# EricLBuehler/mistral.rs

Measured on NVIDIA H100. Metric: decode_tok_s, higher is better.
Workload: dtype int8 activations x 4/6-bit ggml blocks (dp4a), f32 accumulate, bf16 I/O

## Files before the change

mistral.rs_b200/csrc/common.cuh:

```cuda
#pragma once
#include <cuda_bf16.h>
#include <cuda_fp16.h>
#include <cuda_runtime.h>
#include <stdint.h>

#define MRS_WARP 32

enum : int {
  MRS_Q4_0 = 2, MRS_Q4_1 = 3, MRS_Q5_0 = 6, MRS_Q5_1 = 7, MRS_Q8_0 = 8, MRS_Q8_1 = 9,
  MRS_Q2_K = 10, MRS_Q3_K = 11, MRS_Q4_K = 12, MRS_Q5_K = 13, MRS_Q6_K = 14
};
enum : int { MRS_F16 = 0, MRS_BF16 = 1, MRS_F32 = 2 };

struct __align__(4) block_q8_1 {
  __half2 ds;
  int8_t qs[32];
};
static_assert(sizeof(block_q8_1) == 36, "q8_1 layout");

__device__ __forceinline__ float warp_sum(float x) {
#pragma unroll
  for (int m = 16; m > 0; m >>= 1) x += __shfl_xor_sync(0xffffffffu, x, m);
  return x;
}
__device__ __forceinline__ float warp_max(float x) {
#pragma unroll
  for (int m = 16; m > 0; m >>= 1) x = fmaxf(x, __shfl_xor_sync(0xffffffffu, x, m));
  return x;
}

__device__ __forceinline__ uint32_t smem_u32(const void *p) {
  return (uint32_t)__cvta_generic_to_shared(p);
}

__device__ __forceinline__ float load_act(const void *p, int64_t i, int dtype) {
  if (dtype == MRS_BF16) return __bfloat162float(((const __nv_bfloat16 *)p)[i]);
  if (dtype == MRS_F16) return __half2float(((const __half *)p)[i]);
  return ((const float *)p)[i];
}
__device__ __forceinline__ void store_act(void *p, int64_t i, float v, int dtype) {
  if (dtype == MRS_BF16) ((__nv_bfloat16 *)p)[i] = __float2bfloat16_rn(v);
  else if (dtype == MRS_F16) ((__half *)p)[i] = __float2half_rn(v);
  else ((float *)p)[i] = v;
}
__device__ __forceinline__ void load_act8(const void *p, int64_t i, int dtype, float *out) {
  if (dtype == MRS_BF16) {
    const uint4 v = *(const uint4 *)((const __nv_bfloat16 *)p + i);
    const __nv_bfloat162 *h = (const __nv_bfloat162 *)&v;
#pragma unroll
    for (int k = 0; k < 4; k++) { const float2 t = __bfloat1622float2(h[k]); out[2 * k] = t.x; out[2 * k + 1] = t.y; }
  } else if (dtype == MRS_F16) {
    const uint4 v = *(const uint4 *)((const __half *)p + i);
    const __half2 *h = (const __half2 *)&v;
#pragma unroll
    for (int k = 0; k < 4; k++) { const float2 t = __half22float2(h[k]); out[2 * k] = t.x; out[2 * k + 1] = t.y; }
  } else {
    const float4 a = *(const float4 *)((const float *)p + i), b = *(const float4 *)((const float *)p + i + 4);
    out[0] = a.x; out[1] = a.y; out[2] = a.z; out[3] = a.w; out[4] = b.x; out[5] = b.y; out[6] = b.z; out[7] = b.w;
  }
}
__device__ __forceinline__ void unpack_act8(const uint4 &v, int dtype, float *out) {
  if (dtype == MRS_BF16) {
    const __nv_bfloat162 *h = (const __nv_bfloat162 *)&v;
#pragma unroll
    for (int k = 0; k < 4; k++) { const float2 t = __bfloat1622float2(h[k]); out[2 * k] = t.x; out[2 * k + 1] = t.y; }
  } else {
    const __half2 *h = (const __half2 *)&v;
#pragma unroll
    for (int k = 0; k < 4; k++) { const float2 t = __half22float2(h[k]); out[2 * k] = t.x; out[2 * k + 1] = t.y; }
  }
}
__device__ __forceinline__ float round_act(float v, int dtype) {
  if (dtype == MRS_BF16) return __bfloat162float(__float2bfloat16_rn(v));
  if (dtype == MRS_F16) return __half2float(__float2half_rn(v));
  return v;
}

__device__ __forceinline__ float glu_activation(float x, int act) {
  switch (act) {
  case 1: {
    const float x3 = x * x * x;
    const float inner = 0.7978845608f * (x + 0.044715f * x3);
    float th;
    asm("tanh.approx.f32 %0, %1;" : "=f"(th) : "f"(inner));
    return 0.5f * x * (1.0f + th);
  }
  case 2: return fmaxf(x, 0.0f);
  case 3: return x * normcdff(x);
  case 4: return __fdividef(1.0f, 1.0f + __expf(-x));
  case 0:
  default: return __fdividef(x, 1.0f + __expf(-x));
  }
}

__device__ __forceinline__ void mbar_init(uint64_t *bar, uint32_t count) {
  asm volatile("mbarrier.init.shared::cta.b64 [%0], %1;" ::"r"(smem_u32(bar)), "r"(count));
}
__device__ __forceinline__ void fence_mbar_init() {
  asm volatile("fence.mbarrier_init.release.cluster;" ::: "memory");
}
__device__ __forceinline__ void fence_proxy_async() {
  asm volatile("fence.proxy.async.shared::cta;" ::: "memory");
}
__device__ __forceinline__ void mbar_arrive(uint64_t *bar) {
  asm volatile("mbarrier.arrive.shared::cta.b64 _, [%0];" ::"r"(smem_u32(bar)) : "memory");
}
__device__ __forceinline__ void mbar_arrive_expect_tx(uint64_t *bar, uint32_t bytes) {
  asm volatile("mbarrier.arrive.expect_tx.shared::cta.b64 _, [%0], %1;" ::"r"(smem_u32(bar)),
               "r"(bytes)
               : "memory");
}
__device__ __forceinline__ void mbar_wait(uint64_t *bar, uint32_t parity) {
  asm volatile(
      "{\n\t"
      ".reg .pred P1;\n\t"
      "WAIT_LOOP:\n\t"
      "mbarrier.try_wait.parity.shared::cta.b64 P1, [%0], %1;\n\t"
      "@P1 bra.uni WAIT_DONE;\n\t"
      "bra.uni WAIT_LOOP;\n\t"
      "WAIT_DONE:\n\t"
      "}" ::"r"(smem_u32(bar)),
      "r"(parity)
      : "memory");
}
__device__ __forceinline__ void bulk_g2s(void *dst_smem, const void *src_gmem, uint32_t bytes,
                                         uint64_t *bar) {
  asm volatile(
      "cp.async.bulk.shared::cluster.global.mbarrier::complete_tx::bytes [%0], [%1], %2, [%3];" ::
          "r"(smem_u32(dst_smem)),
      "l"(src_gmem), "r"(bytes), "r"(smem_u32(bar))
      : "memory");
}
__device__ __forceinline__ void pdl_wait() { asm volatile("griddepcontrol.wait;" ::: "memory"); }
__device__ __forceinline__ void pdl_launch_dependents() {
  asm volatile("griddepcontrol.launch_dependents;" ::: "memory");
}

__device__ __forceinline__ uint4 lds128(uint32_t saddr) {
  uint4 v;
  asm volatile("ld.shared.v4.u32 {%0, %1, %2, %3}, [%4];" : "=r"(v.x), "=r"(v.y), "=r"(v.z), "=r"(v.w) : "r"(saddr));
  return v;
}
__device__ __forceinline__ uint32_t lds32(uint32_t saddr) {
  uint32_t v;
  asm volatile("ld.shared.u32 %0, [%1];" : "=r"(v) : "r"(saddr));
  return v;
}
__device__ __forceinline__ uint32_t lds_u16s(uint32_t saddr) {
  uint16_t v;
  asm volatile("ld.shared.u16 %0, [%1];" : "=h"(v) : "r"(saddr));
  return (uint32_t)v;
}
__device__ __forceinline__ void sts128(uint32_t saddr, const uint4 &v) {
  asm volatile("st.shared.v4.u32 [%0], {%1, %2, %3, %4};" ::"r"(saddr), "r"(v.x), "r"(v.y), "r"(v.z), "r"(v.w) : "memory");
}
__device__ __forceinline__ void sts32(uint32_t saddr, uint32_t v) {
  asm volatile("st.shared.u32 [%0], %1;" ::"r"(saddr), "r"(v) : "memory");
}

__device__ __forceinline__ uint32_t lds_u32_unaligned(const uint8_t *p) {
  const uintptr_t a = (uintptr_t)p;
  const uint32_t *w = (const uint32_t *)(a & ~(uintptr_t)3);
  const uint32_t sh = (uint32_t)(a & 3) * 8;
  return __funnelshift_r(w[0], w[1], sh);
}
template <int N>
__device__ __forceinline__ void lds_words_unaligned(const uint8_t *p, uint32_t (&out)[N]) {
  const uintptr_t a = (uintptr_t)p;
  const uint32_t *w = (const uint32_t *)(a & ~(uintptr_t)3);
  const uint32_t sh = (uint32_t)(a & 3) * 8;
  uint32_t t[N + 1];
#pragma unroll
  for (int i = 0; i <= N; i++) t[i] = w[i];
#pragma unroll
  for (int i = 0; i < N; i++) out[i] = __funnelshift_r(t[i], t[i + 1], sh);
}
__device__ __forceinline__ uint32_t lds_u16(const uint8_t *p) {
  return *(const uint16_t *)p;
}

__device__ __forceinline__ float half_bits_to_float(uint32_t h16) {
  return __half2float(__ushort_as_half((unsigned short)h16));
}
```

mistral.rs_b200/csrc/decoder.cu:

```cuda
#include "common.cuh"
#include "dequant.cuh"
#include "mrs_b200_model.h"

#include <stdio.h>

extern "C" int mrs_mmvq_fused(int ggml_type, int mode, int dt, const void *w0, const void *w1, const void *w2,
                              const void *x, const void *norm_w, float eps, const void *residual, void *dst0,
                              void *dst1, void *dst2, int K, int n0, int n1, int n2, int b_size, int activation,
                              int pdl, void *stream);
extern "C" int mrs_mmvq_fused_qkv_mixed(int type_qk, int type_v, int dt, const void *wq, const void *wk, const void *wv,
                                        const void *x, const void *norm_w, float eps, void *q, void *k, void *v,
                                        int K, int nq, int nk, int nv, int b_size, int pdl, void *stream);
extern "C" void rotary_embedding_positions(void *query, void *key, void *cos_cache, void *sin_cache, void *positions,
                                           int32_t is_neox, int32_t head_size, int64_t num_tokens, int32_t rot_dim,
                                           int32_t seq_len, int32_t num_heads, int32_t num_kv_heads,
                                           int64_t query_stride, int64_t key_stride, uint32_t dtype, int64_t stream);
extern "C" void reshape_and_cache_flashinfer(void *key, void *value, void *key_cache, void *value_cache,
                                             int64_t *slot_mapping, int32_t num_tokens, int32_t num_heads,
                                             int32_t head_size, int32_t block_size, int32_t key_stride,
                                             int32_t value_stride, float k_scale, float v_scale, uint32_t dtype,
                                             uint32_t cache_dtype, cudaStream_t stream);
extern "C" int32_t mrs_paged_decode_fused(void *q, void *k_new, void *v_new, void *key_cache, void *value_cache,
                                          const void *rope_cos, const void *rope_sin, const int32_t *positions,
                                          const int64_t *slot_mapping, const int32_t *kv_indptr,
                                          const int32_t *kv_indices, const int32_t *kv_last_page_len,
                                          const int32_t *request_indices, const int32_t *kv_tile_indices,
                                          const int32_t *o_indptr, const int32_t *kv_chunk_size_ptr,
                                          const uint8_t *block_valid_mask, void *o, void *tmp_v, float *tmp_s,
                                          int32_t *counters, int32_t batch_size, int32_t padded_batch_size,
                                          int32_t num_qo_heads, int32_t num_kv_heads, int32_t head_size,
                                          int32_t page_size, float sm_scale, uint32_t dtype, int32_t pdl,
                                          void *stream);
extern "C" int32_t flashinfer_decode(void *q, void *key_cache, void *value_cache, const int32_t *kv_indptr,
                                     const int32_t *kv_indices, const int32_t *kv_last_page_len,
                                     const int32_t *request_indices, const int32_t *kv_tile_indices,
                                     const int32_t *o_indptr, const int32_t *kv_chunk_size_ptr,
                                     const bool *block_valid_mask, void *o, void *tmp_v, void *tmp_s,
                                     int32_t batch_size, int32_t padded_batch_size, int32_t num_qo_heads,
                                     int32_t num_kv_heads, int32_t head_size, int32_t page_size, int32_t q_stride_n,
                                     int32_t q_stride_h, float sm_scale, int32_t window_left, float logits_soft_cap,
                                     float k_scale, float v_scale, uint32_t dtype, uint32_t cache_dtype,
                                     cudaStream_t stream);

namespace mrs {

__global__ void embedding_gather_kernel(int type, const uint8_t *__restrict__ table, int cols,
                                        const int32_t *__restrict__ ids, void *__restrict__ out, int act_dtype) {
  const int row = ids[blockIdx.x];
  const int be = blk_elems(type), bb = blk_bytes(type);
  const uint8_t *rp = table + (size_t)row * (cols / be) * bb;
  for (int i = threadIdx.x; i < cols; i += blockDim.x)
    store_act(out, (int64_t)blockIdx.x * cols + i, dequant_elem(type, rp + (size_t)(i / be) * bb, i % be), act_dtype);
}

__device__ __forceinline__ unsigned long long pack_key(float v, int idx) {
  unsigned int b = __float_as_uint(v);
  b = (b & 0x80000000u) ? ~b : (b | 0x80000000u);
  return ((unsigned long long)b << 32) | (unsigned int)(0xFFFFFFFFu - (unsigned int)idx);
}
__global__ void argmax_kernel(const void *__restrict__ logits, int cols, int act_dtype, int32_t *__restrict__ out,
                              unsigned long long *__restrict__ keys, unsigned int *__restrict__ counts, int pdl) {
  __shared__ unsigned long long sk[32];
  if (pdl) pdl_wait();
  const int row = blockIdx.y;
  const int64_t base = (int64_t)row * cols;
  unsigned long long best = 0ull;
  for (int i = blockIdx.x * blockDim.x + threadIdx.x; i < cols; i += gridDim.x * blockDim.x) {
    const unsigned long long k = pack_key(load_act(logits, base + i, act_dtype), i);
    best = k > best ? k : best;
  }
#pragma unroll
  for (int m = 16; m > 0; m >>= 1) {
    const unsigned long long o = __shfl_xor_sync(0xffffffffu, best, m);
    best = o > best ? o : best;
  }
  const int w = threadIdx.x >> 5, l = threadIdx.x & 31;
  if (l == 0) sk[w] = best;
  __syncthreads();
  if (w == 0) {
    best = (l < (blockDim.x >> 5)) ? sk[l] : 0ull;
#pragma unroll
    for (int m = 16; m > 0; m >>= 1) {
      const unsigned long long o = __shfl_xor_sync(0xffffffffu, best, m);
      best = o > best ? o : best;
    }
    if (l == 0) {
      atomicMax(&keys[row], best);
      __threadfence();
      const unsigned int done = atomicAdd(&counts[row], 1u);
      if (done == gridDim.x - 1) {
        __threadfence();
        const unsigned long long k = atomicExch(&keys[row], 0ull);
        out[row] = (int32_t)(0xFFFFFFFFu - (unsigned int)(k & 0xFFFFFFFFull));
        counts[row] = 0u;
      }
    }
  }
}

__global__ void add_residual_kernel(void *__restrict__ dst, const void *__restrict__ res, int64_t n, int dt) {
  const int64_t i = (int64_t)blockIdx.x * blockDim.x + threadIdx.x;
  if (i < n) store_act(dst, i, load_act(dst, i, dt) + load_act(res, i, dt), dt);
}

struct ArCtxDev {
  int world, rank;
  const uint8_t *peer_base[8];
  uint32_t *flags_local;
  unsigned long long flags_off, slot_off[2];
  uint32_t *seq;
  unsigned long long ll_off, ll_slot_stride, ll_src_stride;
};
__global__ void __launch_bounds__(1024) tp_allreduce_residual_kernel(const ArCtxDev c, int slot, const void *__restrict__ residual,
                                                                     void *__restrict__ out, int count, int dt, int pdl) {
  __shared__ uint32_t s_seq;
  if (pdl && threadIdx.x == 0) pdl_launch_dependents();
  if (pdl) pdl_wait();
  if (threadIdx.x == 0) {
    const uint32_t seq = *c.seq + 1u;
    *c.seq = seq;
    __threadfence_system();
    for (int r = 0; r < c.world; r++) {
      uint32_t *flag = (uint32_t *)(c.peer_base[r] + c.flags_off) + c.rank;
      asm volatile("st.release.sys.global.u32 [%0], %1;" ::"l"(flag), "r"(seq) : "memory");
    }
    for (int r = 0; r < c.world; r++) {
      uint32_t v;
      do {
        asm volatile("ld.acquire.sys.global.u32 %0, [%1];" : "=r"(v) : "l"(c.flags_local + r) : "memory");
      } while ((int32_t)(v - seq) < 0);
    }
    s_seq = seq;
  }
  __syncthreads();
  for (int i = threadIdx.x * 8; i < count; i += blockDim.x * 8) {
    float acc[8] = {0.f, 0.f, 0.f, 0.f, 0.f, 0.f, 0.f, 0.f};
    for (int r = 0; r < c.world; r++) {
      const uint4 raw = __ldcv((const uint4 *)(c.peer_base[r] + c.slot_off[slot]) + (i >> 3));
      float v[8];
      unpack_act8(raw, dt, v);
#pragma unroll
      for (int k = 0; k < 8; k++) acc[k] += v[k];
    }
    float res[8];
    load_act8(residual, i, dt, res);
#pragma unroll
    for (int k = 0; k < 8; k++) store_act(out, (int64_t)i + k, round_act(acc[k], dt) + res[k], dt);
  }
}

__global__ void __launch_bounds__(1024) tp_allreduce_ll_kernel(const ArCtxDev c, int slot, const void *__restrict__ partial,
                                                               const void *__restrict__ residual, void *__restrict__ out, int count,
                                                               int dt, int pdl) {
  if (pdl && threadIdx.x == 0) pdl_launch_dependents();
  if (pdl) pdl_wait();
  const uint32_t seq = *(volatile const uint32_t *)c.seq + 1u;
  const bool dead = *(volatile const uint32_t *)(c.seq + 1) != 0u;
  __syncthreads();
  if (threadIdx.x == 0) *(volatile uint32_t *)c.seq = seq;
  const unsigned long long area = c.ll_off + (unsigned long long)slot * c.ll_slot_stride;
  const int npairs = count >> 1;
  for (int i = threadIdx.x; i < npairs; i += blockDim.x) {
    const uint32_t mine = ((const uint32_t *)partial)[i];
    for (int r = 0; r < c.world; r++) {
      if (r == c.rank) continue;
      uint2 *dst = (uint2 *)(c.peer_base[r] + area + (unsigned long long)c.rank * c.ll_src_stride) + i;
      asm volatile("st.volatile.global.v2.u32 [%0], {%1, %2};" ::"l"(dst), "r"(mine), "r"(seq) : "memory");
    }
  }
  for (int i = threadIdx.x; i < npairs; i += blockDim.x) {
    const uint32_t mine = ((const uint32_t *)partial)[i];
    float a0 = 0.f, a1 = 0.f;
    for (int r = 0; r < c.world; r++) {
      uint32_t w = mine;
      if (r != c.rank) {
        const uint2 *src = (const uint2 *)(c.peer_base[c.rank] + area + (unsigned long long)r * c.ll_src_stride) + i;
        uint32_t fl, spins = 0;
        const long long t0 = clock64();
        for (;;) {
          asm volatile("ld.volatile.global.v2.u32 {%0, %1}, [%2];" : "=r"(w), "=r"(fl) : "l"(src) : "memory");
          if (fl == seq || dead) break;
          if ((++spins & 1023u) == 0u &&
              (clock64() - t0 > 500000000ll || *(volatile const uint32_t *)(c.seq + 1) != 0u)) { c.seq[1] = 1u; break; }
        }
      }
      float v0, v1;
      if (dt == MRS_BF16) { const float2 f = __bfloat1622float2(*(const __nv_bfloat162 *)&w); v0 = f.x; v1 = f.y; }
      else { const float2 f = __half22float2(*(const __half2 *)&w); v0 = f.x; v1 = f.y; }
      a0 += v0; a1 += v1;
    }
    const float r0 = load_act(residual, 2 * (int64_t)i, dt), r1 = load_act(residual, 2 * (int64_t)i + 1, dt);
    store_act(out, 2 * (int64_t)i, round_act(a0, dt) + r0, dt);
    store_act(out, 2 * (int64_t)i + 1, round_act(a1, dt) + r1, dt);
  }
}

constexpr int ADV_MAX_BATCH = 256;
__global__ void decode_advance_kernel(const int32_t *__restrict__ block_tables, int max_blocks,
                                      int32_t *__restrict__ context_lens, int batch, int bs, int split_pages,
                                      int padded_tiles, int max_pos, int32_t *positions, int64_t *slot_mapping,
                                      int32_t *kv_indptr, int32_t *kv_indices, int32_t *kv_last_page_len,
                                      int32_t *request_indices, int32_t *kv_tile_indices, int32_t *o_indptr,
                                      int32_t *kv_chunk_size, uint8_t *block_valid_mask, int32_t *error_flag) {
  __shared__ int s_nb[ADV_MAX_BATCH], s_chunks[ADV_MAX_BATCH], s_indptr[ADV_MAX_BATCH + 1], s_oind[ADV_MAX_BATCH + 1];
  const int cap = min(max_blocks * bs, max_pos > 0 ? max_pos : max_blocks * bs);
  for (int b = threadIdx.x; b < batch; b += blockDim.x) {
    int pos = context_lens[b];
    const bool full = pos >= cap;
    if (full) { pos = cap - 1; if (error_flag != nullptr) atomicOr(error_flag, 1); }
    const int ctx = pos + 1;
    context_lens[b] = ctx;
    positions[b] = pos;
    slot_mapping[b] = full ? (int64_t)-1 : (int64_t)block_tables[(int64_t)b * max_blocks + pos / bs] * bs + pos % bs;
    const int nb = (ctx + bs - 1) / bs;
    s_nb[b] = nb;
    kv_last_page_len[b] = ctx - (nb - 1) * bs;
    s_chunks[b] = (split_pages > 0) ? ((nb < 1 ? 1 : nb) + split_pages - 1) / split_pages : 1;
  }
  __syncthreads();
  if (threadIdx.x == 0) {
    int nnz = 0, tiles = 0;
    s_indptr[0] = 0; s_oind[0] = 0;
    for (int b = 0; b < batch; b++) {
      nnz += s_nb[b];
      tiles = min(tiles + s_chunks[b], padded_tiles);
      s_indptr[b + 1] = nnz; s_oind[b + 1] = tiles;
    }
    kv_chunk_size[0] = (split_pages > 0 ? split_pages : 1) * bs;
  }
  __syncthreads();
  const int tiles = s_oind[batch];
  for (int b = threadIdx.x; b <= batch; b += blockDim.x) { kv_indptr[b] = s_indptr[b]; o_indptr[b] = s_oind[b]; }
  for (int b = 0; b < batch; b++) {
    const int t0 = s_oind[b], nt = s_oind[b + 1] - t0;
    for (int t = threadIdx.x; t < nt; t += blockDim.x) { request_indices[t0 + t] = b; kv_tile_indices[t0 + t] = t; }
    const int p0 = s_indptr[b], nb = s_indptr[b + 1] - p0;
    for (int i = threadIdx.x; i < nb; i += blockDim.x) kv_indices[p0 + i] = block_tables[(int64_t)b * max_blocks + i];
  }
  for (int t = threadIdx.x; t < padded_tiles; t += blockDim.x) {
    block_valid_mask[t] = t < tiles ? 1 : 0;
    if (t >= tiles) { request_indices[t] = 0; kv_tile_indices[t] = 0; }
  }
}

}

using namespace mrs;

extern "C" int32_t mrs_embedding_gather(int32_t ggml_type, const void *table, int32_t cols, const int32_t *ids,
                                        int32_t n, void *out, int32_t act_dtype, void *stream) {
  if (n <= 0) return 0;
  if (blk_bytes(ggml_type) == 0 || cols % blk_elems(ggml_type)) return (int32_t)cudaErrorInvalidValue;
  embedding_gather_kernel<<<n, 256, 0, (cudaStream_t)stream>>>(ggml_type, (const uint8_t *)table, cols, ids, out, act_dtype);
  return (int32_t)cudaGetLastError();
}

extern "C" int32_t mrs_argmax(const void *logits, int32_t rows, int32_t cols, int32_t act_dtype, int32_t *out,
                              void *scratch, int32_t pdl, void *stream) {
  if (rows <= 0) return 0;
  if (scratch == nullptr) return (int32_t)cudaErrorInvalidValue;
  unsigned long long *keys = (unsigned long long *)scratch;
  unsigned int *counts = (unsigned int *)(keys + rows);
  int chunks = (cols + 4095) / 4096;
  if (chunks > 64) chunks = 64;
  cudaLaunchConfig_t cfg = {};
  cfg.gridDim = dim3(chunks, rows); cfg.blockDim = dim3(256); cfg.stream = (cudaStream_t)stream;
  cudaLaunchAttribute attr[1];
  attr[0].id = cudaLaunchAttributeProgrammaticStreamSerialization;
  attr[0].val.programmaticStreamSerializationAllowed = 1;
  cfg.attrs = attr; cfg.numAttrs = pdl ? 1 : 0;
  return (int32_t)cudaLaunchKernelEx(&cfg, argmax_kernel, logits, (int)cols, (int)act_dtype, out, keys, counts, (int)pdl);
}

extern "C" int32_t mrs_decode_advance(const int32_t *block_tables, int32_t max_blocks_per_seq, int32_t *context_lens,
                                      int32_t batch, int32_t block_size, int32_t split_pages, int32_t padded_tiles,
                                      int32_t *positions, int64_t *slot_mapping, int32_t *kv_indptr,
                                      int32_t *kv_indices, int32_t *kv_last_page_len, int32_t *request_indices,
                                      int32_t *kv_tile_indices, int32_t *o_indptr, int32_t *kv_chunk_size,
                                      uint8_t *block_valid_mask, int32_t max_pos, int32_t *error_flag, void *stream) {
  if (batch < 1 || batch > ADV_MAX_BATCH || max_blocks_per_seq < 1 || block_size < 1) return (int32_t)cudaErrorInvalidValue;
  decode_advance_kernel<<<1, 256, 0, (cudaStream_t)stream>>>(block_tables, max_blocks_per_seq, context_lens, batch,
                                                             block_size, split_pages, padded_tiles, max_pos, positions,
                                                             slot_mapping, kv_indptr, kv_indices, kv_last_page_len,
                                                             request_indices, kv_tile_indices, o_indptr, kv_chunk_size,
                                                             block_valid_mask, error_flag);
  return (int32_t)cudaGetLastError();
}

extern "C" int32_t mrs_tp_allreduce_residual(const mrs_tp_ctx *ctx, int32_t slot, const void *residual, void *out,
                                             int32_t count, int32_t dtype, int32_t pdl, void *stream) {
  if (ctx == nullptr || ctx->world < 1 || ctx->world > 8 || (slot & ~1) || count % 8 || (dtype != MRS_F16 && dtype != MRS_BF16))
    return (int32_t)cudaErrorInvalidValue;
  ArCtxDev c = {};
  c.world = ctx->world; c.rank = ctx->rank;
  for (int r = 0; r < ctx->world; r++) c.peer_base[r] = (const uint8_t *)ctx->peer_base[r];
  c.flags_off = (unsigned long long)ctx->flags_offset;
  c.slot_off[0] = (unsigned long long)ctx->slot_offset[0]; c.slot_off[1] = (unsigned long long)ctx->slot_offset[1];
  c.flags_local = (uint32_t *)((uint8_t *)ctx->peer_base[ctx->rank] + ctx->flags_offset);
  c.seq = (uint32_t *)ctx->seq_counter;
  c.ll_off = (unsigned long long)ctx->ll_offset; c.ll_slot_stride = (unsigned long long)ctx->ll_slot_stride;
  c.ll_src_stride = (unsigned long long)ctx->ll_src_stride;
  if (ctx->ll_offset != 0) {
    if ((int64_t)count * 4 > ctx->ll_src_stride) return (int32_t)cudaErrorInvalidValue;
    int th = (count / 2 + 31) / 32 * 32;
    if (th > 1024) th = 1024;
    cudaLaunchConfig_t cfg = {};
    cfg.gridDim = dim3(1); cfg.blockDim = dim3(th); cfg.stream = (cudaStream_t)stream;
    cudaLaunchAttribute attr[1];
    attr[0].id = cudaLaunchAttributeProgrammaticStreamSerialization;
    attr[0].val.programmaticStreamSerializationAllowed = 1;
    cfg.attrs = attr; cfg.numAttrs = pdl ? 1 : 0;
    const void *partial = (const uint8_t *)ctx->peer_base[ctx->rank] + ctx->slot_offset[slot];
    return (int32_t)cudaLaunchKernelEx(&cfg, tp_allreduce_ll_kernel, c, (int)slot, partial, residual, out, (int)count, (int)dtype, (int)pdl);
  }
  int threads = (count / 8 + 31) / 32 * 32;
  if (threads > 1024) threads = 1024;
  if (threads < 32) threads = 32;
  cudaLaunchConfig_t cfg = {};
  cfg.gridDim = dim3(1); cfg.blockDim = dim3(threads); cfg.stream = (cudaStream_t)stream;
  cudaLaunchAttribute attr[1];
  attr[0].id = cudaLaunchAttributeProgrammaticStreamSerialization;
  attr[0].val.programmaticStreamSerializationAllowed = 1;
  cfg.attrs = attr; cfg.numAttrs = pdl ? 1 : 0;
  return (int32_t)cudaLaunchKernelEx(&cfg, tp_allreduce_residual_kernel, c, (int)slot, residual, out, (int)count, (int)dtype, (int)pdl);
}

#define MRS_TRY(expr)                                  \
  do {                                                 \
    const int _e = (int)(expr);                        \
    if (_e != 0) {                                     \
      fprintf(stderr, "mrs_b200: %s -> cudaError %d\n", #expr, _e); \
      return _e;                                       \
    }                                                  \
  } while (0)

extern "C" int32_t mrs_llama_decode_step(const mrs_llama_step *s, void *stream) {
  const int dt = s->act_dtype, B = s->batch, H = s->hidden, pdl = s->pdl;
  const int nq = s->n_heads * s->head_dim, nkv = s->n_kv_heads * s->head_dim;
  cudaStream_t st = (cudaStream_t)stream;
  if (B < 1 || B > 8) return (int32_t)cudaErrorInvalidValue;
  const bool do_attn = !(s->skip_mask & 1), do_gemv = !(s->skip_mask & 2);

  MRS_TRY(mrs_embedding_gather(s->tok_embd.ggml_type, s->tok_embd.data, H, s->token_ids, B, s->x, dt, stream));
  void *hidden = s->x, *hidden2 = s->x2;
  for (int l = 0; l < s->n_layers; l++) {
    const mrs_llama_layer &L = s->layers[l];
    if (!do_gemv) {
    } else if (L.wq.ggml_type != L.wk.ggml_type) {
      MRS_TRY(mrs_mmvq_fused(L.wq.ggml_type, 0, dt, L.wq.data, nullptr, nullptr, hidden, L.attn_norm, s->rms_eps,
                             nullptr, s->q, nullptr, nullptr, H, nq, 0, 0, B, 0, pdl, stream));
      MRS_TRY(mrs_mmvq_fused(L.wk.ggml_type, 0, dt, L.wk.data, nullptr, nullptr, hidden, L.attn_norm, s->rms_eps,
                             nullptr, s->k, nullptr, nullptr, H, nkv, 0, 0, B, 0, pdl, stream));
      MRS_TRY(mrs_mmvq_fused(L.wv.ggml_type, 0, dt, L.wv.data, nullptr, nullptr, hidden, L.attn_norm, s->rms_eps,
                             nullptr, s->v, nullptr, nullptr, H, nkv, 0, 0, B, 0, pdl, stream));
    } else if (L.wk.ggml_type == L.wv.ggml_type) {
      MRS_TRY(mrs_mmvq_fused(L.wq.ggml_type, 2, dt, L.wq.data, L.wk.data, L.wv.data, hidden, L.attn_norm, s->rms_eps,
                             nullptr, s->q, s->k, s->v, H, nq, nkv, nkv, B, 0, pdl, stream));
    } else {
      MRS_TRY(mrs_mmvq_fused(L.wq.ggml_type, 2, dt, L.wq.data, L.wk.data, nullptr, hidden, L.attn_norm, s->rms_eps,
                             nullptr, s->q, s->k, nullptr, H, nq, nkv, 0, B, 0, pdl, stream));
      MRS_TRY(mrs_mmvq_fused(L.wv.ggml_type, 0, dt, L.wv.data, nullptr, nullptr, hidden, L.attn_norm, s->rms_eps,
                             nullptr, s->v, nullptr, nullptr, H, nkv, 0, 0, B, 0, pdl, stream));
    }
    if (do_attn && s->fused_attention) {
      MRS_TRY(mrs_paged_decode_fused(s->q, s->k, s->v, L.k_cache, L.v_cache, s->rope_cos, s->rope_sin, s->positions,
                                     s->slot_mapping, s->kv_indptr, s->kv_indices, s->kv_last_page_len,
                                     s->request_indices, s->kv_tile_indices, s->o_indptr, s->kv_chunk_size,
                                     s->block_valid_mask, s->attn_out, s->padded_tiles > B ? s->tmp_v : nullptr,
                                     s->padded_tiles > B ? s->tmp_s : nullptr, s->attn_counters, B, s->padded_tiles,
                                     s->n_heads, s->n_kv_heads, s->head_dim, s->block_size, s->sm_scale, (uint32_t)dt,
                                     pdl | (s->rope_neox ? 0 : 2), stream));
    } else if (do_attn) {
    rotary_embedding_positions(s->q, s->k, (void *)s->rope_cos, (void *)s->rope_sin, s->positions, s->rope_neox,
                               s->head_dim, B, s->head_dim / 2, 0, s->n_heads, s->n_kv_heads, nq, nkv, (uint32_t)dt,
                               (int64_t)stream);
    reshape_and_cache_flashinfer(s->k, s->v, L.k_cache, L.v_cache, s->slot_mapping, B, s->n_kv_heads, s->head_dim,
                                 s->block_size, nkv, nkv, 1.f, 1.f, (uint32_t)dt, (uint32_t)dt, st);
    MRS_TRY(flashinfer_decode(s->q, L.k_cache, L.v_cache, s->kv_indptr, s->kv_indices, s->kv_last_page_len,
                              s->request_indices, s->kv_tile_indices, s->o_indptr, s->kv_chunk_size,
                              (const bool *)s->block_valid_mask, s->attn_out, s->padded_tiles > B ? s->tmp_v : nullptr,
                              s->padded_tiles > B ? s->tmp_s : nullptr, B, s->padded_tiles, s->n_heads, s->n_kv_heads,
                              s->head_dim, s->block_size, nq, s->head_dim, s->sm_scale, -1, 0.f, 1.f, 1.f,
                              (uint32_t)dt, (uint32_t)dt, st));
    }
    if (!do_gemv) continue;
    if (s->tp != nullptr && s->tp->world > 1) {
      void *part = (uint8_t *)s->tp->peer_base[s->tp->rank] + s->tp->slot_offset[0];
      MRS_TRY(mrs_mmvq_fused(L.wo.ggml_type, 0, dt, L.wo.data, nullptr, nullptr, s->attn_out, nullptr, 0.f, nullptr,
                             part, nullptr, nullptr, nq, H, 0, 0, B, 0, pdl, stream));
      MRS_TRY(mrs_tp_allreduce_residual(s->tp, 0, hidden, hidden2, B * H, dt, pdl, stream));
    } else if (s->all_reduce == nullptr) {
      MRS_TRY(mrs_mmvq_fused(L.wo.ggml_type, 0, dt, L.wo.data, nullptr, nullptr, s->attn_out, nullptr, 0.f, hidden,
                             hidden2, nullptr, nullptr, nq, H, 0, 0, B, 0, pdl, stream));
    } else {
      MRS_TRY(mrs_mmvq_fused(L.wo.ggml_type, 0, dt, L.wo.data, nullptr, nullptr, s->attn_out, nullptr, 0.f, nullptr,
                             hidden2, nullptr, nullptr, nq, H, 0, 0, B, 0, pdl, stream));
      s->all_reduce(hidden2, (int64_t)B * H, dt, stream, s->all_reduce_user);
      add_residual_kernel<<<(unsigned)(((int64_t)B * H + 255) / 256), 256, 0, st>>>(hidden2, hidden, (int64_t)B * H, dt);
    }
    if (L.w_gate.ggml_type != L.w_up.ggml_type || L.w_gate.rows != L.w_up.rows) return (int32_t)cudaErrorInvalidValue;
    MRS_TRY(mrs_mmvq_fused(L.w_gate.ggml_type, 1, dt, L.w_gate.data, L.w_up.data, nullptr, hidden2, L.ffn_norm,
                           s->rms_eps, nullptr, s->act, nullptr, nullptr, H, L.w_gate.rows, L.w_gate.rows, 0, B, 0,
                           pdl, stream));
    if (s->tp != nullptr && s->tp->world > 1) {
      void *part = (uint8_t *)s->tp->peer_base[s->tp->rank] + s->tp->slot_offset[1];
      MRS_TRY(mrs_mmvq_fused(L.w_down.ggml_type, 0, dt, L.w_down.data, nullptr, nullptr, s->act, nullptr, 0.f, nullptr,
                             part, nullptr, nullptr, L.w_down.cols, H, 0, 0, B, 0, pdl, stream));
      MRS_TRY(mrs_tp_allreduce_residual(s->tp, 1, hidden2, hidden, B * H, dt, pdl, stream));
    } else if (s->all_reduce == nullptr) {
      MRS_TRY(mrs_mmvq_fused(L.w_down.ggml_type, 0, dt, L.w_down.data, nullptr, nullptr, s->act, nullptr, 0.f, hidden2,
                             hidden, nullptr, nullptr, L.w_down.cols, H, 0, 0, B, 0, pdl, stream));
    } else {
      MRS_TRY(mrs_mmvq_fused(L.w_down.ggml_type, 0, dt, L.w_down.data, nullptr, nullptr, s->act, nullptr, 0.f, nullptr,
                             hidden, nullptr, nullptr, L.w_down.cols, H, 0, 0, B, 0, pdl, stream));
      s->all_reduce(hidden, (int64_t)B * H, dt, stream, s->all_reduce_user);
      add_residual_kernel<<<(unsigned)(((int64_t)B * H + 255) / 256), 256, 0, st>>>(hidden, hidden2, (int64_t)B * H, dt);
    }
  }
  if (do_gemv)
  MRS_TRY(mrs_mmvq_fused(s->lm_head.ggml_type, 0, dt, s->lm_head.data, nullptr, nullptr, hidden, s->final_norm,
                         s->rms_eps, nullptr, s->logits, nullptr, nullptr, H, s->vocab, 0, 0, B, 0, pdl, stream));
  MRS_TRY(mrs_argmax(s->logits, B, s->vocab, dt, s->out_token, s->argmax_scratch, pdl, stream));
  return 0;
}
```

mistral.rs_b200/csrc/mmvq.cu:

```cuda
#include "mmvq_types.cuh"

#include <stdio.h>

namespace mrs {

constexpr int SSW = 8;

constexpr int MAX_STAGES = 12;

enum { MODE_PLAIN = 0, MODE_GLU = 1, MODE_QKV = 2 };

__device__ __forceinline__ uint4 sel_u4(bool first, const uint4 &a, const uint4 &b) {
  return make_uint4(first ? a.x : b.x, first ? a.y : b.y, first ? a.z : b.z, first ? a.w : b.w);
}

#ifdef MRS_TIMELINE
__device__ __forceinline__ unsigned long long gtimer() {
  unsigned long long t;
  asm volatile("mov.u64 %0, %%globaltimer;" : "=l"(t));
  return t;
}
#define MRS_STAMP(i) do { if (p.dbg != nullptr) p.dbg[(size_t)blockIdx.x * 16 + (i)] = gtimer(); } while (0)
#else
#define MRS_STAMP(i) do { } while (0)
#endif
enum { X_Q8_1 = 0, X_RAW = 1 };

struct MmvqParams {
  const uint8_t *w[3];
  void *dst[3];
  int nrows[3];
  const void *x;
  const void *norm_w;
  const void *residual;
  float eps;
  int xkind, xdtype;
  int K, stride_col_y, stride_col_dst, ncols;
  int mode, activation, dst_dtype;
  int nstages, vrows, pdl, flags;
#ifdef MRS_TIMELINE
  unsigned long long *dbg;
#endif
};

template <int T, int NCW, int UPLX = QT<T>::UPL> struct Geo {
  using Q = QT<T>;
  static constexpr int SLOTS = 2 * NCW;
  static constexpr int UPL = UPLX;
  static constexpr int SEG_UNITS = 32 * UPL;
  static constexpr int SEG_BLOCKS = SEG_UNITS / Q::UPB;
  static constexpr int SEG_BYTES = SEG_BLOCKS * Q::BYTES;
  static constexpr int SLOT_BYTES = (SEG_BYTES + 30 + 15) & ~15;
  static constexpr int STAGE_BYTES = SLOTS * SLOT_BYTES;
  static constexpr int XU_BYTES = 32 + 4 * Q::AUX;
  static constexpr int NBL = (Q::UPB == 1) ? 32 : (SEG_BLOCKS < 32 ? SEG_BLOCKS : 32);
  static constexpr int CPS = (Q::UPB == 1) ? 1 : 32 / NBL;
  static_assert(Q::UPB == 1 || (NBL * CPS == 32 && CPS * UPL == Q::UPB), "segment geometry");
};

template <int T, int UPL> __device__ __forceinline__ int unit_to_pos(int blk, int c) {
  using G = Geo<T, 8, UPL>;
  if constexpr (QT<T>::UPB == 1) {
    return blk;
  } else {
    const int s = blk / G::SEG_BLOCKS, bl = blk - s * G::SEG_BLOCKS;
    return s * G::SEG_UNITS + (c / G::CPS) * 32 + bl + G::NBL * (c % G::CPS);
  }
}
template <int T, int UPL> __device__ __forceinline__ void pos_to_unit(int pos, int &blk, int &c) {
  using G = Geo<T, 8, UPL>;
  if constexpr (QT<T>::UPB == 1) {
    blk = pos; c = 0;
  } else {
    const int s = pos / G::SEG_UNITS, r = pos - s * G::SEG_UNITS;
    const int ui = r >> 5, lane = r & 31;
    blk = s * G::SEG_BLOCKS + (lane % G::NBL);
    c = ui * G::CPS + lane / G::NBL;
  }
}

__device__ __forceinline__ void resolve_row(const MmvqParams &p, int vrow, int which, int &m, int &row) {
  if (p.mode == MODE_QKV) {
    if (vrow < p.nrows[0]) { m = 0; row = vrow; }
    else if (vrow < p.nrows[0] + p.nrows[1]) { m = 1; row = vrow - p.nrows[0]; }
    else { m = 2; row = vrow - p.nrows[0] - p.nrows[1]; }
  } else if (p.mode == MODE_GLU) {
    m = which; row = vrow;
  } else {
    m = 0; row = vrow;
  }
}

struct YGlobal {
  const block_q8_1 *y;
  __device__ __forceinline__ float d(int j) const { return __low2float(y[j].ds); }
  __device__ __forceinline__ float s(int j) const { return __high2float(y[j].ds); }
};
struct YSmem {
  const float2 *ds;
  __device__ __forceinline__ float d(int j) const { return ds[j].x; }
  __device__ __forceinline__ float s(int j) const { return ds[j].y; }
};

__device__ __forceinline__ void quantize_block_q8_1(const float *v, int8_t *q, float &d_out, float &s_out) {
  float amax = 0.f;
#pragma unroll
  for (int i = 0; i < 32; i++) amax = fmaxf(amax, fabsf(v[i]));
  float s[16];
#pragma unroll
  for (int i = 0; i < 16; i++) s[i] = v[i] + v[i + 16];
#pragma unroll
  for (int m = 8; m > 0; m >>= 1) {
#pragma unroll
    for (int i = 0; i < m; i++) s[i] = s[i] + s[i + m];
  }
  const float d = __fdividef(amax, 127.0f);
#pragma unroll
  for (int i = 0; i < 32; i++) q[i] = (amax == 0.0f) ? (int8_t)0 : (int8_t)roundf(__fdividef(v[i], d));
  d_out = __half2float(__float2half_rn(d));
  s_out = __half2float(__float2half_rn(s[0]));
}

template <int T, int NCOLS, bool FAST, int NCW, int UPL = QT<T>::UPL>
__device__ __forceinline__ void mmvq_body(const MmvqParams &p, const int cta, const int ncta) {
  using Q = QT<T>;
  using G = Geo<T, NCW, UPL>;
  constexpr int SLOTS = 2 * NCW;
  extern __shared__ __align__(128) uint8_t smem[];

  const int tid = threadIdx.x;
  const int warp = tid >> 5, lane = tid & 31;
  const int nblocks = p.K / Q::QK;
  const int nseg = (nblocks + G::SEG_BLOCKS - 1) / G::SEG_BLOCKS;
  const int npos = nseg * G::SEG_UNITS;
  const int row_bytes = nblocks * Q::BYTES;
  const int nst = p.nstages;

  uint64_t *full = (uint64_t *)smem;
  uint64_t *empty = full + MAX_STAGES;
  const uint32_t off_xq0 = 256;
  const uint32_t off_xq1 = off_xq0 + (uint32_t)NCOLS * npos * 16;
  const uint32_t off_xa = off_xq1 + (uint32_t)NCOLS * npos * 16;
  const uint32_t off_ring = (off_xa + (uint32_t)NCOLS * npos * Q::AUX * 4 + 127u) & ~127u;
  int4 *xq0 = (int4 *)(smem + off_xq0);
  int4 *xq1 = (int4 *)(smem + off_xq1);
  float *xa = (float *)(smem + off_xa);
  uint8_t *ring = smem + off_ring;

  if (tid == 0) {
    MRS_STAMP(0);
    for (int i = 0; i < nst; i++) { mbar_init(&full[i], 32); mbar_init(&empty[i], NCW); }
    fence_mbar_init();
  }
  __syncthreads();
  if (tid == 0) MRS_STAMP(1);

  const int vr0 = (int)((long long)p.vrows * cta / ncta);
  const int vr1 = (int)((long long)p.vrows * (cta + 1) / ncta);
  const int P = (p.mode == MODE_GLU) ? NCW : SLOTS;

  if (warp == NCW) {
    if (p.pdl) pdl_launch_dependents();
    int stage = 0, phase = 0;
    const int slot = lane;
    for (int base = vr0; base < vr1; base += P) {
      const uint8_t *rowp = nullptr;
      if (slot < SLOTS) {
        const int vrow = (p.mode == MODE_GLU) ? base + (slot >> 1) : base + slot;
        if (vrow < vr1) {
          int m, row;
          resolve_row(p, vrow, slot & 1, m, row);
          rowp = p.w[m] + (size_t)row * row_bytes;
        }
      }
      for (int s = 0; s < nseg; s++) {
        mbar_wait(&empty[stage], phase ^ 1);
        if (rowp != nullptr) {
          const int off = s * G::SEG_BYTES;
          const int len = min(G::SEG_BYTES, row_bytes - off);
          const uintptr_t a = (uintptr_t)(rowp + off);
          const uintptr_t a0 = a & ~(uintptr_t)15;
          const uint32_t bytes = (uint32_t)(((a + len + 15) & ~(uintptr_t)15) - a0);
          mbar_arrive_expect_tx(&full[stage], bytes);
          bulk_g2s(ring + (uint32_t)stage * G::STAGE_BYTES + (uint32_t)slot * G::SLOT_BYTES, (const void *)a0, bytes, &full[stage]);
        } else {
          mbar_arrive(&full[stage]);
        }
        if (lane == 0 && base == vr0 && s == 0) MRS_STAMP(2);
        if (++stage == nst) { stage = 0; phase ^= 1; }
      }
    }
    if (lane == 0) MRS_STAMP(10);
    return;
  }

  const int ctid = tid;
  constexpr int NCT = NCW * 32;
  constexpr int SST = SSW * 32;
  const bool reg16 = p.xkind == X_RAW && p.xdtype != MRS_F32;
  uint4 nwr0 = make_uint4(0u, 0u, 0u, 0u), nwr1 = nwr0;
  if (p.xkind == X_RAW && p.norm_w != nullptr) {
    if (reg16) {
      if (ctid < (p.K >> 3)) nwr0 = __ldg((const uint4 *)p.norm_w + ctid);
      if (NCW == SSW && ctid + NCT < (p.K >> 3)) nwr1 = __ldg((const uint4 *)p.norm_w + ctid + NCT);
    }
    if (!reg16 || (p.K >> 3) > 2 * NCT) {
      const int nbytes = p.K * ((p.xdtype == MRS_F32) ? 4 : 2);
      for (int off = ctid * 128; off < nbytes; off += NCT * 128)
        asm volatile("prefetch.global.L1 [%0];" ::"l"((const char *)p.norm_w + off));
    }
  }
  if (p.pdl) pdl_wait();
  if (tid == 0) MRS_STAMP(3);
  if (p.xkind == X_Q8_1) {
    const block_q8_1 *y = (const block_q8_1 *)p.x;
    for (int idx = ctid; idx < NCOLS * npos; idx += NCT) {
      const int col = idx / npos, pos = idx - col * npos;
      int blk, c;
      pos_to_unit<T, UPL>(pos, blk, c);
      int q[8];
      float a[Q::AUX];
      if (col < p.ncols && blk < nblocks) {
        const block_q8_1 *yb = y + (size_t)col * p.stride_col_y + (size_t)blk * (Q::QK / 32);
#pragma unroll
        for (int w = 0; w < 8; w++) {
          const int e = Q::x_elem(c, w);
          q[w] = *(const int *)(yb[e >> 5].qs + (e & 31));
        }
        Q::aux(q, c, YGlobal{yb}, a);
      } else {
#pragma unroll
        for (int w = 0; w < 8; w++) q[w] = 0;
#pragma unroll
        for (int i = 0; i < Q::AUX; i++) a[i] = 0.f;
      }
      xq0[idx] = make_int4(q[0], q[1], q[2], q[3]);
      xq1[idx] = make_int4(q[4], q[5], q[6], q[7]);
#pragma unroll
      for (int i = 0; i < Q::AUX; i++) xa[(size_t)idx * Q::AUX + i] = a[i];
    }
  } else {
    float *red = (float *)(smem + 192);
    const int nchunks = p.K >> 3;
    const int nchunks_w = (nchunks + 31) & ~31;
    for (int col = 0; col < NCOLS; col++) {
      const bool live = col < p.ncols;
      float inv_rms = 1.0f;
      uint4 xr0 = make_uint4(0u, 0u, 0u, 0u), xr1 = xr0;
      if (reg16 && live) {
        const uint4 *xc = (const uint4 *)((const uint16_t *)p.x + (int64_t)col * p.K);
        if (ctid < nchunks) xr0 = xc[ctid];
        if (ctid < SST && ctid + SST < nchunks) xr1 = xc[ctid + SST];
      }
      if (p.norm_w != nullptr && live) {
        float ss = 0.f;
        int i0 = ctid * 8;
        if (ctid >= SST) {
          i0 = p.K;
        } else if (reg16) {
          float v[8];
          unpack_act8(xr0, p.xdtype, v);
#pragma unroll
          for (int e = 0; e < 8; e++) ss = fmaf(v[e], v[e], ss);
          unpack_act8(xr1, p.xdtype, v);
#pragma unroll
          for (int e = 0; e < 8; e++) ss = fmaf(v[e], v[e], ss);
          i0 += 2 * SST * 8;
        }
        for (int i = i0; i < p.K; i += SST * 8) {
          float v[8];
          load_act8(p.x, (int64_t)col * p.K + i, p.xdtype, v);
#pragma unroll
          for (int k = 0; k < 8; k++) ss = fmaf(v[k], v[k], ss);
        }
        ss = warp_sum(ss);
        asm volatile("bar.sync 1, %0;" ::"n"(NCT));
        if (lane == 0 && warp < SSW) red[warp] = ss;
        asm volatile("bar.sync 1, %0;" ::"n"(NCT));
        float tot = 0.f;
#pragma unroll
        for (int i = 0; i < SSW; i++) tot += red[i];
        inv_rms = rsqrtf(tot / (float)p.K + p.eps);
      }
      if (tid == 0) MRS_STAMP(4);
      int4 *c0 = xq0 + (size_t)col * npos, *c1 = xq1 + (size_t)col * npos;
      float *ca = xa + (size_t)col * npos * Q::AUX;
      int it = 0;
#pragma unroll 1
      for (int ch = ctid; ch < nchunks_w; ch += NCT, it++) {
        const bool ok = ch < nchunks;
        const bool inreg = reg16 && (it == 0 || (it == 1 && NCW == SSW));
        float v[8];
        if (ok && live) {
          if (inreg) unpack_act8(sel_u4(it == 0, xr0, xr1), p.xdtype, v);
          else load_act8(p.x, (int64_t)col * p.K + ch * 8, p.xdtype, v);
          if (p.norm_w != nullptr) {
            float wv[8];
            if (inreg) unpack_act8(sel_u4(it == 0, nwr0, nwr1), p.xdtype, wv);
            else load_act8(p.norm_w, ch * 8, p.xdtype, wv);
#pragma unroll
            for (int i = 0; i < 8; i++) v[i] = round_act(v[i] * inv_rms * wv[i], p.xdtype);
          }
        } else {
#pragma unroll
          for (int i = 0; i < 8; i++) v[i] = 0.f;
        }
        float am = 0.f;
#pragma unroll
        for (int i = 0; i < 8; i++) am = fmaxf(am, fabsf(v[i]));
        am = fmaxf(am, __shfl_xor_sync(0xffffffffu, am, 1));
        am = fmaxf(am, __shfl_xor_sync(0xffffffffu, am, 2));
        float bsum = 0.f;
        if constexpr (Q::NEEDS_SUM) {
          float t[8];
#pragma unroll
          for (int i = 0; i < 8; i++) t[i] = v[i] + __shfl_xor_sync(0xffffffffu, v[i], 2);
#pragma unroll
          for (int i = 0; i < 8; i++) t[i] = t[i] + __shfl_xor_sync(0xffffffffu, t[i], 1);
#pragma unroll
          for (int m = 4; m > 0; m >>= 1) {
#pragma unroll
            for (int i = 0; i < m; i++) t[i] = t[i] + t[i + m];
          }
          bsum = __half2float(__float2half_rn(t[0]));
        }
        const float d = __fdividef(am, 127.0f);
        uint32_t wq[2] = {0u, 0u};
#pragma unroll
        for (int i = 0; i < 8; i++) {
          const int qi = (am == 0.0f) ? 0 : (int)(int8_t)roundf(__fdividef(v[i], d));
          wq[i >> 2] |= (uint32_t)(qi & 0xff) << (8 * (i & 3));
        }
        const int isum8 = __dp4a((int)wq[0], 0x01010101, __dp4a((int)wq[1], 0x01010101, 0));
        const int isum16 = isum8 + __shfl_xor_sync(0xffffffffu, isum8, 1);
        if (ok) {
          const int e0 = ch * 8;
          const int blk = e0 / Q::QK, e = e0 - blk * Q::QK;
          int c, hi, w8;
          Q::chunk_dest(e, c, hi, w8);
          const int pos = unit_to_pos<T, UPL>(blk, c);
          *((int2 *)((hi ? c1 : c0) + pos) + w8) = make_int2((int)wq[0], (int)wq[1]);
          Q::chunk_aux(e, __half2float(__float2half_rn(d)), bsum, isum8, isum16, ca + (size_t)pos * Q::AUX);
        }
      }
    }
  }
  asm volatile("bar.sync 1, %0;" ::"n"(NCT));

  if (tid == 0) MRS_STAMP(6);
  int stage = 0, phase = 0;
  const int lblk = lane % G::NBL;
  const int lsub = lane / G::NBL;
  for (int base = vr0; base < vr1; base += P) {
    bool valid[2];
    int mm[2], rr[2];
    uint32_t ph[2];
#pragma unroll
    for (int r = 0; r < 2; r++) {
      int vrow = (p.mode == MODE_GLU) ? base + warp : base + 2 * warp + r;
      valid[r] = vrow < vr1;
      if (!valid[r]) vrow = vr1 - 1;
      resolve_row(p, vrow, r, mm[r], rr[r]);
      ph[r] = (uint32_t)((uintptr_t)(p.w[mm[r]] + (size_t)rr[r] * row_bytes) & 15);
    }
    float acc[2][NCOLS];
#pragma unroll
    for (int r = 0; r < 2; r++)
#pragma unroll
      for (int j = 0; j < NCOLS; j++) acc[r][j] = 0.f;

    for (int s = 0; s < nseg; s++) {
      mbar_wait(&full[stage], phase);
      if (tid == 0 && base == vr0 && s == 0) MRS_STAMP(7);
      const uint8_t *st = ring + (uint32_t)stage * G::STAGE_BYTES + (uint32_t)(2 * warp) * G::SLOT_BYTES;
      const uint32_t sp = (uint32_t)(s * G::SEG_BYTES) & 15u;
      const uint8_t *wp0 = st + ((ph[0] + sp) & 15u) + lblk * Q::BYTES;
      const uint8_t *wp1 = st + G::SLOT_BYTES + ((ph[1] + sp) & 15u) + lblk * Q::BYTES;
      const bool live = (s * G::SEG_BLOCKS + lblk) < nblocks;
#pragma unroll
      for (int ui = 0; ui < G::UPL; ui++) {
        const int c = (Q::UPB == 1) ? 0 : ui * G::CPS + lsub;
        const uint32_t boff = (Q::UPB == 1) ? (uint32_t)(ui * 32 * Q::BYTES) : 0u;
        const bool ulive = (Q::UPB == 1) ? (s * G::SEG_BLOCKS + ui * 32 + lblk) < nblocks : live;
        if (ulive && (valid[0] || valid[1])) {
          typename Q::W w0, w1;
          Q::template load<FAST>(wp0 + boff, c, w0);
          Q::template load<FAST>(wp1 + boff, c, w1);
          const int pos = s * G::SEG_UNITS + ui * 32 + lane;
#pragma unroll
          for (int j = 0; j < NCOLS; j++) {
            const int idx = j * npos + pos;
            const int4 q0 = xq0[idx], q1 = xq1[idx];
            const int xq[8] = {q0.x, q0.y, q0.z, q0.w, q1.x, q1.y, q1.z, q1.w};
            float a[Q::AUX];
            if constexpr (Q::AUX == 4) {
              const float4 t = *(const float4 *)(xa + (size_t)idx * 4);
              a[0] = t.x; a[1] = t.y; a[2] = t.z; a[3] = t.w;
            } else if constexpr (Q::AUX == 2) {
              const float2 t = *(const float2 *)(xa + (size_t)idx * 2);
              a[0] = t.x; a[1] = t.y;
            } else if constexpr (Q::AUX == 8) {
              const float4 t0 = *(const float4 *)(xa + (size_t)idx * 8), t1 = *(const float4 *)(xa + (size_t)idx * 8 + 4);
              a[0] = t0.x; a[1] = t0.y; a[2] = t0.z; a[3] = t0.w; a[4] = t1.x; a[5] = t1.y; a[6] = t1.z; a[7] = t1.w;
            } else {
#pragma unroll
              for (int i = 0; i < Q::AUX; i++) a[i] = xa[(size_t)idx * Q::AUX + i];
            }
            acc[0][j] += Q::dot(w0, xq, a, c);
            acc[1][j] += Q::dot(w1, xq, a, c);
          }
        }
      }
      __syncwarp();
      if (lane == 0) mbar_arrive(&empty[stage]);
      if (++stage == nst) { stage = 0; phase ^= 1; }
    }

    if (tid == 0 && base + P >= vr1) MRS_STAMP(8);
#pragma unroll
    for (int r = 0; r < 2; r++)
#pragma unroll
      for (int j = 0; j < NCOLS; j++) acc[r][j] = warp_sum(acc[r][j]);

    if (lane == 0) {
      if (p.mode == MODE_GLU) {
        if (valid[0]) {
#pragma unroll
          for (int j = 0; j < NCOLS; j++) {
            if (j < p.ncols) {
              const float g = round_act(acc[0][j], p.dst_dtype);
              const float up = round_act(acc[1][j], p.dst_dtype);
              const float act = round_act(glu_activation(g, p.activation), p.dst_dtype);
              store_act(p.dst[0], (int64_t)j * p.stride_col_dst + rr[0], act * up, p.dst_dtype);
            }
          }
        }
      } else {
#pragma unroll
        for (int r = 0; r < 2; r++) {
          if (!valid[r]) continue;
          const int nr = p.nrows[mm[r]];
          const int64_t cs = (p.mode == MODE_QKV) ? nr : p.stride_col_dst;
#pragma unroll
          for (int j = 0; j < NCOLS; j++) {
            if (j < p.ncols) {
              float v = acc[r][j];
              if (p.residual != nullptr) {
                v = round_act(v, p.dst_dtype) + load_act(p.residual, (int64_t)j * cs + rr[r], p.dst_dtype);
              }
              store_act(p.dst[mm[r]], (int64_t)j * cs + rr[r], v, p.dst_dtype);
            }
          }
        }
      }
    }
  }
  if (tid == 0) {
    MRS_STAMP(9);
#ifdef MRS_TIMELINE
    if (p.dbg != nullptr) { p.dbg[(size_t)blockIdx.x * 16 + 15] = gridDim.x; p.dbg[(size_t)blockIdx.x * 16 + 14] = (unsigned long long)p.vrows << 32 | (unsigned)p.K; }
#endif
  }
}

template <int T, int NCOLS, bool FAST, int NCW, int UPL>
__global__ void __launch_bounds__((NCW + 1) * 32, NCOLS == 1 ? 3 : 2) mmvq_stream_kernel(const MmvqParams p) {
  mmvq_body<T, NCOLS, FAST, NCW, UPL>(p, (int)blockIdx.x, (int)gridDim.x);
}

template <int T1, int T2>
__global__ void __launch_bounds__(9 * 32, 2) mmvq_dual_kernel(const MmvqParams pa, const MmvqParams pb, const int g1) {
  if ((int)blockIdx.x < g1) mmvq_body<T1, 1, true, 8>(pa, (int)blockIdx.x, g1);
  else mmvq_body<T2, 1, true, 8>(pb, (int)blockIdx.x - g1, (int)gridDim.x - g1);
}

#ifdef MRS_TIMELINE
static unsigned long long *g_dbg = nullptr;
static int g_dbg_launch = 0, g_dbg_max = 0;
extern "C" int mrs_mmvq_timeline(unsigned long long *buf, int max_launches) {
  const int n = g_dbg_launch;
  g_dbg = buf; g_dbg_max = max_launches; g_dbg_launch = 0;
  return n;
}
#endif
constexpr int MAX_DEVICES = 64;
struct DevInfo { int num_sms, max_smem; };
static DevInfo g_dev[MAX_DEVICES] = {};
static int g_flags = 0;
static long long g_long_min_bytes = 128ll << 20;
static int g_ctas_per_sm = 2;

static const DevInfo &query_device() {
  int dev = 0;
  cudaGetDevice(&dev);
  if (dev < 0 || dev >= MAX_DEVICES) dev = 0;
  DevInfo &d = g_dev[dev];
  if (d.num_sms == 0) {
    int sms = 0, smem = 0;
    cudaDeviceGetAttribute(&sms, cudaDevAttrMultiProcessorCount, dev);
    cudaDeviceGetAttribute(&smem, cudaDevAttrMaxSharedMemoryPerBlockOptin, dev);
    d.max_smem = smem > 0 ? smem : 227 * 1024;
    d.num_sms = sms > 0 ? sms : 132;
  }
  return d;
}

template <int T, int UPL>
static bool plan8(const MmvqParams &p, int ncols, const DevInfo &d, int &nst, size_t &smem, int &ctas_per_sm) {
  using G = Geo<T, 8, UPL>;
  const int nblocks = p.K / QT<T>::QK;
  const int nseg = (nblocks + G::SEG_BLOCKS - 1) / G::SEG_BLOCKS;
  const int npos = nseg * G::SEG_UNITS;
  const size_t xbytes = 256 + (size_t)ncols * npos * G::XU_BYTES + 128;
  ctas_per_sm = (ncols == 1) ? g_ctas_per_sm : (g_ctas_per_sm > 2 ? 2 : g_ctas_per_sm);
  size_t budget = (size_t)d.max_smem / (ctas_per_sm < 2 ? 2 : ctas_per_sm) - 1024;
  const size_t full = (size_t)d.max_smem - 1024;
  nst = MAX_STAGES;
  while (nst > 2 && xbytes + (size_t)nst * G::STAGE_BYTES > budget) nst--;
  smem = xbytes + (size_t)nst * G::STAGE_BYTES;
  if (smem > budget && ctas_per_sm == 3) {
    ctas_per_sm = 2;
    budget = (size_t)d.max_smem / 2 - 1024;
    nst = MAX_STAGES;
    while (nst > 2 && xbytes + (size_t)nst * G::STAGE_BYTES > budget) nst--;
    smem = xbytes + (size_t)nst * G::STAGE_BYTES;
  }
  if (smem > budget) {
    ctas_per_sm = 1;
    while (nst < 4 && xbytes + (size_t)(nst + 1) * G::STAGE_BYTES <= full) nst++;
    smem = xbytes + (size_t)nst * G::STAGE_BYTES;
  }
  return smem <= (size_t)d.max_smem;
}

template <int T, int NCOLS, bool FAST, int UPL>
static cudaError_t launch_one(MmvqParams p, cudaStream_t stream) {
  constexpr int NCW = 8, SLOTS = 2 * NCW;
  const DevInfo &d = query_device();
  int nst, ctas_per_sm;
  size_t smem;
  if (!plan8<T, UPL>(p, NCOLS, d, nst, smem, ctas_per_sm)) return cudaErrorInvalidConfiguration;
  p.nstages = nst;
  p.flags = g_flags;
#ifdef MRS_TIMELINE
  p.dbg = (g_dbg != nullptr && g_dbg_launch < g_dbg_max) ? g_dbg + (size_t)(g_dbg_launch++) * 320 * 16 : nullptr;
#endif
  const int P = (p.mode == MODE_GLU) ? NCW : SLOTS;
  int grid = (p.vrows + P - 1) / P;
  const int max_grid = ctas_per_sm * d.num_sms;
  if (grid > max_grid) grid = max_grid;
  if (grid < 1) grid = 1;
  auto kern = mmvq_stream_kernel<T, NCOLS, FAST, NCW, UPL>;
  cudaFuncSetAttribute(kern, cudaFuncAttributeMaxDynamicSharedMemorySize, d.max_smem);
  cudaLaunchConfig_t cfg = {};
  cfg.gridDim = dim3(grid);
  cfg.blockDim = dim3((NCW + 1) * 32);
  cfg.dynamicSmemBytes = smem;
  cfg.stream = stream;
  cudaLaunchAttribute attr[1];
  attr[0].id = cudaLaunchAttributeProgrammaticStreamSerialization;
  attr[0].val.programmaticStreamSerializationAllowed = 1;
  cfg.attrs = attr;
  cfg.numAttrs = p.pdl ? 1 : 0;
  return cudaLaunchKernelEx(&cfg, kern, p);
}

template <int T> static bool rows_aligned(const MmvqParams &p) {
  using Q = QT<T>;
  const int row_bytes = (p.K / Q::QK) * Q::BYTES;
  bool fast = (row_bytes % Q::WALIGN) == 0;
  for (int m = 0; m < 3; m++)
    if (p.w[m] != nullptr && ((uintptr_t)p.w[m] % Q::WALIGN) != 0) fast = false;
  return fast;
}

template <int T1, int T2>
static cudaError_t launch_dual(MmvqParams pa, MmvqParams pb, cudaStream_t stream) {
  const DevInfo &d = query_device();
  int nsa, nsb, ca, cb;
  size_t sma, smb;
  if (pa.ncols != 1 || pb.ncols != 1 || !rows_aligned<T1>(pa) || !rows_aligned<T2>(pb) ||
      !plan8<T1, QT<T1>::UPL>(pa, 1, d, nsa, sma, ca) || !plan8<T2, QT<T2>::UPL>(pb, 1, d, nsb, smb, cb) || ca < 2 || cb < 2)
    return cudaErrorNotSupported;
  if (ca != 2 || cb != 2) {
    const int keep = g_ctas_per_sm; g_ctas_per_sm = 2;
    const bool ok = plan8<T1, QT<T1>::UPL>(pa, 1, d, nsa, sma, ca) && plan8<T2, QT<T2>::UPL>(pb, 1, d, nsb, smb, cb) && ca == 2 && cb == 2;
    g_ctas_per_sm = keep;
    if (!ok) return cudaErrorNotSupported;
  }
  pa.nstages = nsa; pb.nstages = nsb; pa.flags = pb.flags = g_flags;
#ifdef MRS_TIMELINE
  pa.dbg = (g_dbg != nullptr && g_dbg_launch < g_dbg_max) ? g_dbg + (size_t)(g_dbg_launch++) * 320 * 16 : nullptr;
  pb.dbg = pa.dbg;
#endif
  const int slots = 2 * d.num_sms;
  const int Pa = (pa.mode == MODE_GLU) ? 8 : 16, Pb = (pb.mode == MODE_GLU) ? 8 : 16;
  int ga = (pa.vrows + Pa - 1) / Pa, gb = (pb.vrows + Pb - 1) / Pb;
  if (ga < 1 || gb < 1) return cudaErrorNotSupported;
  if (ga + gb > slots) {
    if (gb > slots / 2) gb = slots / 2;
    if (ga > slots - gb) ga = slots - gb;
  }
  auto kern = mmvq_dual_kernel<T1, T2>;
  cudaFuncSetAttribute(kern, cudaFuncAttributeMaxDynamicSharedMemorySize, d.max_smem);
  cudaLaunchConfig_t cfg = {};
  cfg.gridDim = dim3(ga + gb);
  cfg.blockDim = dim3(9 * 32);
  cfg.dynamicSmemBytes = sma > smb ? sma : smb;
  cfg.stream = stream;
  cudaLaunchAttribute attr[1];
  attr[0].id = cudaLaunchAttributeProgrammaticStreamSerialization;
  attr[0].val.programmaticStreamSerializationAllowed = 1;
  cfg.attrs = attr;
  cfg.numAttrs = pa.pdl ? 1 : 0;
  return cudaLaunchKernelEx(&cfg, kern, pa, pb, ga);
}

static cudaError_t mmvq_dispatch_dual(int t1, const MmvqParams &pa, int t2, const MmvqParams &pb, cudaStream_t stream) {
  if (t1 == MRS_Q4_K && t2 == MRS_Q6_K) return launch_dual<MRS_Q4_K, MRS_Q6_K>(pa, pb, stream);
  if (t1 == MRS_Q5_K && t2 == MRS_Q6_K) return launch_dual<MRS_Q5_K, MRS_Q6_K>(pa, pb, stream);
  if (t1 == MRS_Q4_K && t2 == MRS_Q5_K) return launch_dual<MRS_Q4_K, MRS_Q5_K>(pa, pb, stream);
  return cudaErrorNotSupported;
}

template <int T> struct HasLong { static constexpr bool value = (T == MRS_Q4_K || T == MRS_Q6_K); };

template <int T>
static cudaError_t launch_type(MmvqParams p, cudaStream_t stream) {
  using Q = QT<T>;
  const bool fast = rows_aligned<T>(p);
  const int row_bytes = (p.K / Q::QK) * Q::BYTES;
  size_t wbytes = 0;
  for (int m = 0; m < 3; m++)
    if (p.w[m] != nullptr) wbytes += (size_t)p.nrows[m] * row_bytes;
  const int b = p.ncols;
#define MRS_DISPATCH(NC)                                                                          \
  do {                                                                                            \
    if constexpr (HasLong<T>::value) {                                                            \
      if (fast && NC == 1 && !(g_flags & 8) && wbytes >= (size_t)g_long_min_bytes)                \
        return launch_one<T, NC, true, 2 * Q::UPL>(p, stream);                                    \
    }                                                                                             \
    return fast ? launch_one<T, NC, true, Q::UPL>(p, stream) : launch_one<T, NC, false, Q::UPL>(p, stream); \
  } while (0)
  if (b == 1) { MRS_DISPATCH(1); }
  if (b == 2) { MRS_DISPATCH(2); }
  if (b <= 4) { MRS_DISPATCH(4); }
  MRS_DISPATCH(8);
#undef MRS_DISPATCH
}

cudaError_t mmvq_dispatch(int type, const MmvqParams &p, cudaStream_t stream) {
  if (p.ncols < 1 || p.ncols > 8) return cudaErrorInvalidValue;
  switch (type) {
  case MRS_Q4_0: return launch_type<MRS_Q4_0>(p, stream);
  case MRS_Q4_1: return launch_type<MRS_Q4_1>(p, stream);
  case MRS_Q5_0: return launch_type<MRS_Q5_0>(p, stream);
  case MRS_Q5_1: return launch_type<MRS_Q5_1>(p, stream);
  case MRS_Q8_0: return launch_type<MRS_Q8_0>(p, stream);
  case MRS_Q2_K: return launch_type<MRS_Q2_K>(p, stream);
  case MRS_Q3_K: return launch_type<MRS_Q3_K>(p, stream);
  case MRS_Q4_K: return launch_type<MRS_Q4_K>(p, stream);
  case MRS_Q5_K: return launch_type<MRS_Q5_K>(p, stream);
  case MRS_Q6_K: return launch_type<MRS_Q6_K>(p, stream);
  default: return cudaErrorInvalidValue;
  }
}

template <typename T>
__global__ void quantize_q8_1_kernel(const T *__restrict__ x, block_q8_1 *__restrict__ y, int kx, int kx_padded) {
  const int ix = blockDim.x * blockIdx.x + threadIdx.x;
  if (ix >= kx_padded) return;
  const int iy = blockIdx.y;
  const int64_t ip = (int64_t)iy * kx_padded + ix;
  const int ib = (int)(ip >> 5), iqs = (int)(ip & 31);
  const float xi = (ix < kx) ? (float)x[(int64_t)iy * kx + ix] : 0.0f;
  const float amax = warp_max(fabsf(xi));
  const float sum = warp_sum(xi);
  const float d = __fdividef(amax, 127.0f);
  const int8_t q = (amax == 0.0f) ? (int8_t)0 : (int8_t)roundf(__fdividef(xi, d));
  y[ib].qs[iqs] = q;
  if (iqs == 0) y[ib].ds = __halves2half2(__float2half_rn(d), __float2half_rn(sum));
}

}

using namespace mrs;

static int g_mrs_pdl = 0;

extern "C" void mrs_set_pdl(int enabled) { g_mrs_pdl = enabled; }
extern "C" void mrs_set_mmvq_flags(int f) { g_flags = f & 0xff; if (f >> 8) g_long_min_bytes = (long long)(f >> 8) << 20; }
extern "C" int mrs_mmvq_has_wide(void) { return 0; }
extern "C" void mrs_set_mmvq_ctas_per_sm(int n) { g_ctas_per_sm = n < 1 ? 1 : (n > 3 ? 3 : n); }

static inline void report(cudaError_t e, const char *what) {
  if (e != cudaSuccess) fprintf(stderr, "mrs_b200: %s failed: %s\n", what, cudaGetErrorString(e));
}

#define MRS_Q8_1_LAUNCHER(tag, ctype)                                                          \
  extern "C" void launch_mmvq_gguf_quantize_q8_1_##tag(const void *x, void *vy, int kx,        \
                                                       int kx_padded, int num_rows,            \
                                                       void *stream) {                         \
    dim3 grid((kx_padded + 255) / 256, num_rows, 1);                                           \
    quantize_q8_1_kernel<ctype><<<grid, 256, 0, (cudaStream_t)stream>>>(                       \
        (const ctype *)x, (block_q8_1 *)vy, kx, kx_padded);                                    \
  }
MRS_Q8_1_LAUNCHER(bf16, __nv_bfloat16)
MRS_Q8_1_LAUNCHER(f16, __half)
MRS_Q8_1_LAUNCHER(f32, float)

static void run_plain(int type, int dt, const void *vx, const void *vy, void *dst, int ncols_x, int nrows_x,
                      int stride_col_y, int stride_col_dst, int b_size, void *stream) {
  if (b_size < 1 || b_size > 8) return;
  MmvqParams p = {};
  p.w[0] = (const uint8_t *)vx; p.dst[0] = dst; p.nrows[0] = nrows_x;
  p.x = vy; p.xkind = X_Q8_1; p.K = ncols_x; p.stride_col_y = stride_col_y;
  p.stride_col_dst = stride_col_dst; p.ncols = b_size; p.mode = MODE_PLAIN; p.dst_dtype = dt;
  p.vrows = nrows_x; p.pdl = g_mrs_pdl;
  report(mmvq_dispatch(type, p, (cudaStream_t)stream), "mmvq plain");
}

static void run_glu(int type, int dt, const void *vg, const void *vu, const void *vy, void *dst, int ncols_x,
                    int nrows_x, int stride_col_y, int stride_col_dst, int b_size, int activation, void *stream) {
  if (b_size < 1 || b_size > 8) return;
  MmvqParams p = {};
  p.w[0] = (const uint8_t *)vg; p.w[1] = (const uint8_t *)vu; p.dst[0] = dst; p.nrows[0] = nrows_x; p.nrows[1] = nrows_x;
  p.x = vy; p.xkind = X_Q8_1; p.K = ncols_x; p.stride_col_y = stride_col_y;
  p.stride_col_dst = stride_col_dst; p.ncols = b_size; p.mode = MODE_GLU; p.activation = activation;
  p.dst_dtype = dt; p.vrows = nrows_x; p.pdl = g_mrs_pdl;
  report(mmvq_dispatch(type, p, (cudaStream_t)stream), "mmvq fused_glu");
}

static void run_qkv(int type, int dt, const void *vq, const void *vk, const void *vv, const void *vy, void *qd,
                    void *kd, void *vd, int ncols_x, int nq, int nk, int nv, int stride_col_y, int b_size,
                    void *stream) {
  if (b_size < 1 || b_size > 8) return;
  MmvqParams p = {};
  p.w[0] = (const uint8_t *)vq; p.w[1] = (const uint8_t *)vk; p.w[2] = (const uint8_t *)vv;
  p.dst[0] = qd; p.dst[1] = kd; p.dst[2] = vd; p.nrows[0] = nq; p.nrows[1] = nk; p.nrows[2] = nv;
  p.x = vy; p.xkind = X_Q8_1; p.K = ncols_x; p.stride_col_y = stride_col_y; p.ncols = b_size;
  p.mode = MODE_QKV; p.dst_dtype = dt; p.vrows = nq + nk + nv; p.pdl = g_mrs_pdl;
  report(mmvq_dispatch(type, p, (cudaStream_t)stream), "mmvq fused_qkv");
}

#define MRS_MMVQ_SET(tag, TYPE, dtag, DT)                                                              \
  extern "C" void launch_mmvq_gguf_##tag##_##dtag##_plain(const void *vx, const void *vy, void *dst,   \
      int ncols_x, int nrows_x, int stride_col_y, int stride_col_dst, int b_size, void *stream) {      \
    run_plain(TYPE, DT, vx, vy, dst, ncols_x, nrows_x, stride_col_y, stride_col_dst, b_size, stream);  \
  }                                                                                                    \
  extern "C" void launch_mmvq_gguf_##tag##_##dtag##_fused_glu(const void *vx_gate, const void *vx_up,  \
      const void *vy, void *dst, int ncols_x, int nrows_x, int stride_col_y, int stride_col_dst,       \
      int b_size, int activation, void *stream) {                                                      \
    run_glu(TYPE, DT, vx_gate, vx_up, vy, dst, ncols_x, nrows_x, stride_col_y, stride_col_dst, b_size, \
            activation, stream);                                                                       \
  }                                                                                                    \
  extern "C" void launch_mmvq_gguf_##tag##_##dtag##_fused_qkv(const void *vx_q, const void *vx_k,      \
      const void *vx_v, const void *vy, void *q_dst, void *k_dst, void *v_dst, int ncols_x,            \
      int nrows_q, int nrows_k, int nrows_v, int stride_col_y, int b_size, void *stream) {             \
    run_qkv(TYPE, DT, vx_q, vx_k, vx_v, vy, q_dst, k_dst, v_dst, ncols_x, nrows_q, nrows_k, nrows_v,   \
            stride_col_y, b_size, stream);                                                             \
  }
#define MRS_MMVQ_TYPE(tag, TYPE)            \
  MRS_MMVQ_SET(tag, TYPE, bf16, MRS_BF16)   \
  MRS_MMVQ_SET(tag, TYPE, f16, MRS_F16)     \
  MRS_MMVQ_SET(tag, TYPE, f32, MRS_F32)
MRS_MMVQ_TYPE(q4_0, MRS_Q4_0)
MRS_MMVQ_TYPE(q4_1, MRS_Q4_1)
MRS_MMVQ_TYPE(q5_0, MRS_Q5_0)
MRS_MMVQ_TYPE(q5_1, MRS_Q5_1)
MRS_MMVQ_TYPE(q8_0, MRS_Q8_0)
MRS_MMVQ_TYPE(q2_k, MRS_Q2_K)
MRS_MMVQ_TYPE(q3_k, MRS_Q3_K)
MRS_MMVQ_TYPE(q4_k, MRS_Q4_K)
MRS_MMVQ_TYPE(q5_k, MRS_Q5_K)
MRS_MMVQ_TYPE(q6_k, MRS_Q6_K)

static cudaError_t mmvq_dispatch_dual_entry(int t1, const MmvqParams &pa, int t2, const MmvqParams &pb, cudaStream_t stream);

extern "C" int mrs_mmvq_fused(int ggml_type, int mode, int dt, const void *w0, const void *w1, const void *w2,
                              const void *x, const void *norm_w, float eps, const void *residual,
                              void *dst0, void *dst1, void *dst2, int K, int n0, int n1, int n2,
                              int b_size, int activation, int pdl, void *stream) {
  MmvqParams p = {};
  p.w[0] = (const uint8_t *)w0; p.w[1] = (const uint8_t *)w1; p.w[2] = (const uint8_t *)w2;
  p.dst[0] = dst0; p.dst[1] = dst1; p.dst[2] = dst2;
  p.nrows[0] = n0; p.nrows[1] = n1; p.nrows[2] = n2;
  p.x = x; p.xkind = X_RAW; p.xdtype = dt; p.norm_w = norm_w; p.eps = eps; p.residual = residual;
  p.K = K; p.stride_col_dst = n0; p.ncols = b_size; p.mode = mode; p.activation = activation;
  p.dst_dtype = dt; p.pdl = pdl;
  p.vrows = (mode == MODE_QKV) ? n0 + n1 + n2 : n0;
  return (int)mmvq_dispatch(ggml_type, p, (cudaStream_t)stream);
}

static cudaError_t mmvq_dispatch_dual_entry(int t1, const MmvqParams &pa, int t2, const MmvqParams &pb, cudaStream_t stream) {
  return mrs::mmvq_dispatch_dual(t1, pa, t2, pb, stream);
}

extern "C" int mrs_mmvq_fused_qkv_mixed(int type_qk, int type_v, int dt, const void *wq, const void *wk, const void *wv,
                                        const void *x, const void *norm_w, float eps, void *q, void *k, void *v,
                                        int K, int nq, int nk, int nv, int b_size, int pdl, void *stream) {
  MmvqParams pa = {}, pb = {};
  pa.w[0] = (const uint8_t *)wq; pa.w[1] = (const uint8_t *)wk; pa.dst[0] = q; pa.dst[1] = k;
  pa.nrows[0] = nq; pa.nrows[1] = nk; pa.nrows[2] = 0;
  pa.x = x; pa.xkind = X_RAW; pa.xdtype = dt; pa.norm_w = norm_w; pa.eps = eps;
  pa.K = K; pa.stride_col_dst = nq; pa.ncols = b_size; pa.mode = MODE_QKV; pa.dst_dtype = dt; pa.pdl = pdl;
  pa.vrows = nq + nk;
  pb.w[0] = (const uint8_t *)wv; pb.dst[0] = v; pb.nrows[0] = nv;
  pb.x = x; pb.xkind = X_RAW; pb.xdtype = dt; pb.norm_w = norm_w; pb.eps = eps;
  pb.K = K; pb.stride_col_dst = nv; pb.ncols = b_size; pb.mode = MODE_PLAIN; pb.dst_dtype = dt; pb.pdl = pdl;
  pb.vrows = nv;
  cudaError_t e = (b_size == 1) ? mmvq_dispatch_dual_entry(type_qk, pa, type_v, pb, (cudaStream_t)stream) : cudaErrorNotSupported;
  if (e != cudaErrorNotSupported) return (int)e;
  e = mmvq_dispatch(type_qk, pa, (cudaStream_t)stream);
  if (e != cudaSuccess) return (int)e;
  return (int)mmvq_dispatch(type_v, pb, (cudaStream_t)stream);
}
```

Baseline: 360.1.

## Prefetch next GEMV's weight rows into L2 and stream current weights evict-first

The decode loop now builds the full per-layer list of GEMV calls ahead of time, so each mmvq launch knows the weights of the following GEMV. After finishing its own TMA stream, each CTA's producer warp issues bulk L2 prefetches for the leading rows the next kernel's CTAs will read, capped by a byte budget that is larger before attention. Current weight loads use an evict-first L2 policy so streamed weights do not push out the prefetched data. The aim is to hide DRAM latency at kernel boundaries. The cost is extra host planning, possible L2 contention, and prefetches that only help if they land before the next kernel reads them.

```diff
diff --git a/mistral.rs_b200/csrc/common.cuh b/mistral.rs_b200/csrc/common.cuh
--- a/mistral.rs_b200/csrc/common.cuh
+++ b/mistral.rs_b200/csrc/common.cuh
@@ -131,6 +131,22 @@
       "l"(src_gmem), "r"(bytes), "r"(smem_u32(bar))
       : "memory");
 }
+__device__ __forceinline__ void bulk_g2s_hint(void *dst_smem, const void *src_gmem, uint32_t bytes, uint64_t *bar,
+                                              uint64_t policy) {
+  asm volatile(
+      "cp.async.bulk.shared::cluster.global.mbarrier::complete_tx::bytes.L2::cache_hint [%0], [%1], %2, [%3], %4;" ::
+          "r"(smem_u32(dst_smem)),
+      "l"(src_gmem), "r"(bytes), "r"(smem_u32(bar)), "l"(policy)
+      : "memory");
+}
+__device__ __forceinline__ uint64_t l2_policy_evict_first() {
+  uint64_t pol;
+  asm volatile("createpolicy.fractional.L2::evict_first.b64 %0, 1.0;" : "=l"(pol));
+  return pol;
+}
+__device__ __forceinline__ void bulk_prefetch_l2(const void *src_gmem, uint32_t bytes) {
+  asm volatile("cp.async.bulk.prefetch.L2.global [%0], %1;" ::"l"(src_gmem), "r"(bytes) : "memory");
+}
 __device__ __forceinline__ void pdl_wait() { asm volatile("griddepcontrol.wait;" ::: "memory"); }
 __device__ __forceinline__ void pdl_launch_dependents() {
   asm volatile("griddepcontrol.launch_dependents;" ::: "memory");
diff --git a/mistral.rs_b200/csrc/decoder.cu b/mistral.rs_b200/csrc/decoder.cu
--- a/mistral.rs_b200/csrc/decoder.cu
+++ b/mistral.rs_b200/csrc/decoder.cu
@@ -1,5 +1,6 @@
 #include "common.cuh"
 #include "dequant.cuh"
+#include "mmvq_call.cuh"
 #include "mrs_b200_model.h"
 
 #include <stdio.h>
@@ -334,6 +335,46 @@
     }                                                  \
   } while (0)
 
+static int layer_gemvs(const mrs_llama_step *s, int l, MmvqCall g[5], int *nqkv) {
+  const int dt = s->act_dtype, B = s->batch, H = s->hidden, pdl = s->pdl;
+  const int nq = s->n_heads * s->head_dim, nkv = s->n_kv_heads * s->head_dim;
+  const mrs_llama_layer &L = s->layers[l];
+  void *hidden = s->x, *hidden2 = s->x2;
+  const bool tp = s->tp != nullptr && s->tp->world > 1;
+  auto gemv = [&](int type, int mode, const void *w0, const void *w1, const void *w2, const void *x, const void *norm_w,
+                  float eps, const void *residual, void *d0, void *d1, void *d2, int K, int n0, int n1, int n2) {
+    return MmvqCall{type, mode, dt, {w0, w1, w2}, x, norm_w, eps, residual, {d0, d1, d2}, K, {n0, n1, n2}, B, 0, pdl};
+  };
+  int n = 0;
+  if (L.wq.ggml_type != L.wk.ggml_type) {
+    g[n++] = gemv(L.wq.ggml_type, 0, L.wq.data, nullptr, nullptr, hidden, L.attn_norm, s->rms_eps, nullptr, s->q, nullptr,
+                  nullptr, H, nq, 0, 0);
+    g[n++] = gemv(L.wk.ggml_type, 0, L.wk.data, nullptr, nullptr, hidden, L.attn_norm, s->rms_eps, nullptr, s->k, nullptr,
+                  nullptr, H, nkv, 0, 0);
+    g[n++] = gemv(L.wv.ggml_type, 0, L.wv.data, nullptr, nullptr, hidden, L.attn_norm, s->rms_eps, nullptr, s->v, nullptr,
+                  nullptr, H, nkv, 0, 0);
+  } else if (L.wk.ggml_type == L.wv.ggml_type) {
+    g[n++] = gemv(L.wq.ggml_type, 2, L.wq.data, L.wk.data, L.wv.data, hidden, L.attn_norm, s->rms_eps, nullptr, s->q, s->k,
+                  s->v, H, nq, nkv, nkv);
+  } else {
+    g[n++] = gemv(L.wq.ggml_type, 2, L.wq.data, L.wk.data, nullptr, hidden, L.attn_norm, s->rms_eps, nullptr, s->q, s->k,
+                  nullptr, H, nq, nkv, 0);
+    g[n++] = gemv(L.wv.ggml_type, 0, L.wv.data, nullptr, nullptr, hidden, L.attn_norm, s->rms_eps, nullptr, s->v, nullptr,
+                  nullptr, H, nkv, 0, 0);
+  }
+  *nqkv = n;
+  void *part0 = tp ? (uint8_t *)s->tp->peer_base[s->tp->rank] + s->tp->slot_offset[0] : nullptr;
+  const bool local = !tp && s->all_reduce == nullptr;
+  g[n++] = gemv(L.wo.ggml_type, 0, L.wo.data, nullptr, nullptr, s->attn_out, nullptr, 0.f, local ? hidden : nullptr,
+                tp ? part0 : hidden2, nullptr, nullptr, nq, H, 0, 0);
+  g[n++] = gemv(L.w_gate.ggml_type, 1, L.w_gate.data, L.w_up.data, nullptr, hidden2, L.ffn_norm, s->rms_eps, nullptr,
+                s->act, nullptr, nullptr, H, L.w_gate.rows, L.w_gate.rows, 0);
+  void *part1 = tp ? (uint8_t *)s->tp->peer_base[s->tp->rank] + s->tp->slot_offset[1] : nullptr;
+  g[n++] = gemv(L.w_down.ggml_type, 0, L.w_down.data, nullptr, nullptr, s->act, nullptr, 0.f, local ? hidden2 : nullptr,
+                tp ? part1 : hidden, nullptr, nullptr, L.w_down.cols, H, 0, 0);
+  return n;
+}
+
 extern "C" int32_t mrs_llama_decode_step(const mrs_llama_step *s, void *stream) {
   const int dt = s->act_dtype, B = s->batch, H = s->hidden, pdl = s->pdl;
   const int nq = s->n_heads * s->head_dim, nkv = s->n_kv_heads * s->head_dim;
@@ -343,25 +384,25 @@
 
   MRS_TRY(mrs_embedding_gather(s->tok_embd.ggml_type, s->tok_embd.data, H, s->token_ids, B, s->x, dt, stream));
   void *hidden = s->x, *hidden2 = s->x2;
+  const MmvqCall head = {s->lm_head.ggml_type, 0, dt, {s->lm_head.data, nullptr, nullptr}, hidden, s->final_norm,
+                         s->rms_eps, nullptr, {s->logits, nullptr, nullptr}, H, {s->vocab, 0, 0}, B, 0, pdl};
+  MmvqCall cur[5] = {}, nxt[5] = {}, first = {};
+  int nqkv = 0, nqkv_next = 0;
+  if (s->n_layers > 0) {
+    layer_gemvs(s, 0, cur, &nqkv);
+    first = cur[0];
+  }
   for (int l = 0; l < s->n_layers; l++) {
     const mrs_llama_layer &L = s->layers[l];
-    if (!do_gemv) {
-    } else if (L.wq.ggml_type != L.wk.ggml_type) {
-      MRS_TRY(mrs_mmvq_fused(L.wq.ggml_type, 0, dt, L.wq.data, nullptr, nullptr, hidden, L.attn_norm, s->rms_eps,
-                             nullptr, s->q, nullptr, nullptr, H, nq, 0, 0, B, 0, pdl, stream));
-      MRS_TRY(mrs_mmvq_fused(L.wk.ggml_type, 0, dt, L.wk.data, nullptr, nullptr, hidden, L.attn_norm, s->rms_eps,
-                             nullptr, s->k, nullptr, nullptr, H, nkv, 0, 0, B, 0, pdl, stream));
-      MRS_TRY(mrs_mmvq_fused(L.wv.ggml_type, 0, dt, L.wv.data, nullptr, nullptr, hidden, L.attn_norm, s->rms_eps,
-                             nullptr, s->v, nullptr, nullptr, H, nkv, 0, 0, B, 0, pdl, stream));
-    } else if (L.wk.ggml_type == L.wv.ggml_type) {
-      MRS_TRY(mrs_mmvq_fused(L.wq.ggml_type, 2, dt, L.wq.data, L.wk.data, L.wv.data, hidden, L.attn_norm, s->rms_eps,
-                             nullptr, s->q, s->k, s->v, H, nq, nkv, nkv, B, 0, pdl, stream));
-    } else {
-      MRS_TRY(mrs_mmvq_fused(L.wq.ggml_type, 2, dt, L.wq.data, L.wk.data, nullptr, hidden, L.attn_norm, s->rms_eps,
-                             nullptr, s->q, s->k, nullptr, H, nq, nkv, 0, B, 0, pdl, stream));
-      MRS_TRY(mrs_mmvq_fused(L.wv.ggml_type, 0, dt, L.wv.data, nullptr, nullptr, hidden, L.attn_norm, s->rms_eps,
-                             nullptr, s->v, nullptr, nullptr, H, nkv, 0, 0, B, 0, pdl, stream));
-    }
+    const int ncur = nqkv + 3;
+    const MmvqCall *after = &head;
+    if (l + 1 < s->n_layers) {
+      layer_gemvs(s, l + 1, nxt, &nqkv_next);
+      after = &nxt[0];
+    }
+    auto gemv = [&](int i) { return mmvq_fused_call(cur[i], i + 1 < ncur ? &cur[i + 1] : after, i == nqkv && do_attn, st); };
+    if (do_gemv)
+      for (int i = 0; i < nqkv; i++) MRS_TRY(gemv(i));
     if (do_attn && s->fused_attention) {
       MRS_TRY(mrs_paged_decode_fused(s->q, s->k, s->v, L.k_cache, L.v_cache, s->rope_cos, s->rope_sin, s->positions,
                                      s->slot_mapping, s->kv_indptr, s->kv_indices, s->kv_last_page_len,
@@ -383,43 +424,31 @@
                               s->head_dim, s->block_size, nq, s->head_dim, s->sm_scale, -1, 0.f, 1.f, 1.f,
                               (uint32_t)dt, (uint32_t)dt, st));
     }
-    if (!do_gemv) continue;
+    if (!do_gemv) {
+      for (int i = 0; i < 5; i++) cur[i] = nxt[i];
+      nqkv = nqkv_next;
+      continue;
+    }
+    MRS_TRY(gemv(nqkv));
     if (s->tp != nullptr && s->tp->world > 1) {
-      void *part = (uint8_t *)s->tp->peer_base[s->tp->rank] + s->tp->slot_offset[0];
-      MRS_TRY(mrs_mmvq_fused(L.wo.ggml_type, 0, dt, L.wo.data, nullptr, nullptr, s->attn_out, nullptr, 0.f, nullptr,
-                             part, nullptr, nullptr, nq, H, 0, 0, B, 0, pdl, stream));
       MRS_TRY(mrs_tp_allreduce_residual(s->tp, 0, hidden, hidden2, B * H, dt, pdl, stream));
-    } else if (s->all_reduce == nullptr) {
-      MRS_TRY(mrs_mmvq_fused(L.wo.ggml_type, 0, dt, L.wo.data, nullptr, nullptr, s->attn_out, nullptr, 0.f, hidden,
-                             hidden2, nullptr, nullptr, nq, H, 0, 0, B, 0, pdl, stream));
-    } else {
-      MRS_TRY(mrs_mmvq_fused(L.wo.ggml_type, 0, dt, L.wo.data, nullptr, nullptr, s->attn_out, nullptr, 0.f, nullptr,
-                             hidden2, nullptr, nullptr, nq, H, 0, 0, B, 0, pdl, stream));
+    } else if (s->all_reduce != nullptr) {
       s->all_reduce(hidden2, (int64_t)B * H, dt, stream, s->all_reduce_user);
       add_residual_kernel<<<(unsigned)(((int64_t)B * H + 255) / 256), 256, 0, st>>>(hidden2, hidden, (int64_t)B * H, dt);
     }
     if (L.w_gate.ggml_type != L.w_up.ggml_type || L.w_gate.rows != L.w_up.rows) return (int32_t)cudaErrorInvalidValue;
-    MRS_TRY(mrs_mmvq_fused(L.w_gate.ggml_type, 1, dt, L.w_gate.data, L.w_up.data, nullptr, hidden2, L.ffn_norm,
-                           s->rms_eps, nullptr, s->act, nullptr, nullptr, H, L.w_gate.rows, L.w_gate.rows, 0, B, 0,
-                           pdl, stream));
+    MRS_TRY(gemv(nqkv + 1));
+    MRS_TRY(gemv(nqkv + 2));
     if (s->tp != nullptr && s->tp->world > 1) {
-      void *part = (uint8_t *)s->tp->peer_base[s->tp->rank] + s->tp->slot_offset[1];
-      MRS_TRY(mrs_mmvq_fused(L.w_down.ggml_type, 0, dt, L.w_down.data, nullptr, nullptr, s->act, nullptr, 0.f, nullptr,
-                             part, nullptr, nullptr, L.w_down.cols, H, 0, 0, B, 0, pdl, stream));
       MRS_TRY(mrs_tp_allreduce_residual(s->tp, 1, hidden2, hidden, B * H, dt, pdl, stream));
-    } else if (s->all_reduce == nullptr) {
-      MRS_TRY(mrs_mmvq_fused(L.w_down.ggml_type, 0, dt, L.w_down.data, nullptr, nullptr, s->act, nullptr, 0.f, hidden2,
-                             hidden, nullptr, nullptr, L.w_down.cols, H, 0, 0, B, 0, pdl, stream));
-    } else {
-      MRS_TRY(mrs_mmvq_fused(L.w_down.ggml_type, 0, dt, L.w_down.data, nullptr, nullptr, s->act, nullptr, 0.f, nullptr,
-                             hidden, nullptr, nullptr, L.w_down.cols, H, 0, 0, B, 0, pdl, stream));
+    } else if (s->all_reduce != nullptr) {
       s->all_reduce(hidden, (int64_t)B * H, dt, stream, s->all_reduce_user);
       add_residual_kernel<<<(unsigned)(((int64_t)B * H + 255) / 256), 256, 0, st>>>(hidden, hidden2, (int64_t)B * H, dt);
     }
-  }
-  if (do_gemv)
-  MRS_TRY(mrs_mmvq_fused(s->lm_head.ggml_type, 0, dt, s->lm_head.data, nullptr, nullptr, hidden, s->final_norm,
-                         s->rms_eps, nullptr, s->logits, nullptr, nullptr, H, s->vocab, 0, 0, B, 0, pdl, stream));
+    for (int i = 0; i < 5; i++) cur[i] = nxt[i];
+    nqkv = nqkv_next;
+  }
+  if (do_gemv) MRS_TRY(mmvq_fused_call(head, s->n_layers > 0 ? &first : nullptr, false, st));
   MRS_TRY(mrs_argmax(s->logits, B, s->vocab, dt, s->out_token, s->argmax_scratch, pdl, stream));
   return 0;
 }
diff --git a/mistral.rs_b200/csrc/mmvq.cu b/mistral.rs_b200/csrc/mmvq.cu
--- a/mistral.rs_b200/csrc/mmvq.cu
+++ b/mistral.rs_b200/csrc/mmvq.cu
@@ -1,3 +1,5 @@
+#include "mmvq_call.cuh"
+#include "mmvq_plan.cuh"
 #include "mmvq_types.cuh"
 
 #include <stdio.h>
@@ -5,10 +7,6 @@
 namespace mrs {
 
 constexpr int SSW = 8;
-
-constexpr int MAX_STAGES = 12;
-
-enum { MODE_PLAIN = 0, MODE_GLU = 1, MODE_QKV = 2 };
 
 __device__ __forceinline__ uint4 sel_u4(bool first, const uint4 &a, const uint4 &b) {
   return make_uint4(first ? a.x : b.x, first ? a.y : b.y, first ? a.z : b.z, first ? a.w : b.w);
@@ -38,6 +36,7 @@
   int K, stride_col_y, stride_col_dst, ncols;
   int mode, activation, dst_dtype;
   int nstages, vrows, pdl, flags;
+  MmvqNext next;
 #ifdef MRS_TIMELINE
   unsigned long long *dbg;
 #endif
@@ -47,12 +46,13 @@
   using Q = QT<T>;
   static constexpr int SLOTS = 2 * NCW;
   static constexpr int UPL = UPLX;
-  static constexpr int SEG_UNITS = 32 * UPL;
-  static constexpr int SEG_BLOCKS = SEG_UNITS / Q::UPB;
-  static constexpr int SEG_BYTES = SEG_BLOCKS * Q::BYTES;
-  static constexpr int SLOT_BYTES = (SEG_BYTES + 30 + 15) & ~15;
-  static constexpr int STAGE_BYTES = SLOTS * SLOT_BYTES;
-  static constexpr int XU_BYTES = 32 + 4 * Q::AUX;
+  static constexpr SegGeo S = seg_geo(Q::BYTES, Q::UPB, Q::AUX, UPL, NCW);
+  static constexpr int SEG_UNITS = S.seg_units;
+  static constexpr int SEG_BLOCKS = S.seg_blocks;
+  static constexpr int SEG_BYTES = S.seg_bytes;
+  static constexpr int SLOT_BYTES = S.slot_bytes;
+  static constexpr int STAGE_BYTES = S.stage_bytes;
+  static constexpr int XU_BYTES = S.xu_bytes;
   static constexpr int NBL = (Q::UPB == 1) ? 32 : (SEG_BLOCKS < 32 ? SEG_BLOCKS : 32);
   static constexpr int CPS = (Q::UPB == 1) ? 1 : 32 / NBL;
   static_assert(Q::UPB == 1 || (NBL * CPS == 32 && CPS * UPL == Q::UPB), "segment geometry");
@@ -80,15 +80,7 @@
 }
 
 __device__ __forceinline__ void resolve_row(const MmvqParams &p, int vrow, int which, int &m, int &row) {
-  if (p.mode == MODE_QKV) {
-    if (vrow < p.nrows[0]) { m = 0; row = vrow; }
-    else if (vrow < p.nrows[0] + p.nrows[1]) { m = 1; row = vrow - p.nrows[0]; }
-    else { m = 2; row = vrow - p.nrows[0] - p.nrows[1]; }
-  } else if (p.mode == MODE_GLU) {
-    m = which; row = vrow;
-  } else {
-    m = 0; row = vrow;
-  }
+  plan_resolve_row(p.mode, p.nrows, vrow, which, m, row);
 }
 
 struct YGlobal {
@@ -155,14 +147,15 @@
   __syncthreads();
   if (tid == 0) MRS_STAMP(1);
 
-  const int vr0 = (int)((long long)p.vrows * cta / ncta);
-  const int vr1 = (int)((long long)p.vrows * (cta + 1) / ncta);
-  const int P = (p.mode == MODE_GLU) ? NCW : SLOTS;
+  int vr0, vr1;
+  plan_cta_rows(p.vrows, cta, ncta, vr0, vr1);
+  const int P = plan_rows_per_pass(p.mode, NCW);
 
   if (warp == NCW) {
     if (p.pdl) pdl_launch_dependents();
     int stage = 0, phase = 0;
     const int slot = lane;
+    const uint64_t stream_policy = l2_policy_evict_first();
     for (int base = vr0; base < vr1; base += P) {
       const uint8_t *rowp = nullptr;
       if (slot < SLOTS) {
@@ -177,17 +170,27 @@
         mbar_wait(&empty[stage], phase ^ 1);
         if (rowp != nullptr) {
           const int off = s * G::SEG_BYTES;
-          const int len = min(G::SEG_BYTES, row_bytes - off);
-          const uintptr_t a = (uintptr_t)(rowp + off);
-          const uintptr_t a0 = a & ~(uintptr_t)15;
-          const uint32_t bytes = (uint32_t)(((a + len + 15) & ~(uintptr_t)15) - a0);
+          uintptr_t a0;
+          uint32_t bytes;
+          plan_granules((uintptr_t)(rowp + off), (uint32_t)min(G::SEG_BYTES, row_bytes - off), a0, bytes);
           mbar_arrive_expect_tx(&full[stage], bytes);
-          bulk_g2s(ring + (uint32_t)stage * G::STAGE_BYTES + (uint32_t)slot * G::SLOT_BYTES, (const void *)a0, bytes, &full[stage]);
+          bulk_g2s_hint(ring + (uint32_t)stage * G::STAGE_BYTES + (uint32_t)slot * G::SLOT_BYTES, (const void *)a0, bytes,
+                        &full[stage], stream_policy);
         } else {
           mbar_arrive(&full[stage]);
         }
         if (lane == 0 && base == vr0 && s == 0) MRS_STAMP(2);
         if (++stage == nst) { stage = 0; phase ^= 1; }
+      }
+    }
+    for (int j = cta; j < p.next.grid && p.next.lead > 0; j += ncta) {
+      int nvr0;
+      const int n = plan_prefetch_items(p.next, j, nvr0);
+      for (int i = lane; i < n; i += 32) {
+        uintptr_t a0;
+        uint32_t bytes;
+        plan_prefetch_item(p.next, nvr0, i, a0, bytes);
+        bulk_prefetch_l2((const void *)a0, bytes);
       }
     }
     if (lane == 0) MRS_STAMP(10);
@@ -506,56 +509,27 @@
 }
 
 template <int T, int UPL>
-static bool plan8(const MmvqParams &p, int ncols, const DevInfo &d, int &nst, size_t &smem, int &ctas_per_sm) {
-  using G = Geo<T, 8, UPL>;
-  const int nblocks = p.K / QT<T>::QK;
-  const int nseg = (nblocks + G::SEG_BLOCKS - 1) / G::SEG_BLOCKS;
-  const int npos = nseg * G::SEG_UNITS;
-  const size_t xbytes = 256 + (size_t)ncols * npos * G::XU_BYTES + 128;
-  ctas_per_sm = (ncols == 1) ? g_ctas_per_sm : (g_ctas_per_sm > 2 ? 2 : g_ctas_per_sm);
-  size_t budget = (size_t)d.max_smem / (ctas_per_sm < 2 ? 2 : ctas_per_sm) - 1024;
-  const size_t full = (size_t)d.max_smem - 1024;
-  nst = MAX_STAGES;
-  while (nst > 2 && xbytes + (size_t)nst * G::STAGE_BYTES > budget) nst--;
-  smem = xbytes + (size_t)nst * G::STAGE_BYTES;
-  if (smem > budget && ctas_per_sm == 3) {
-    ctas_per_sm = 2;
-    budget = (size_t)d.max_smem / 2 - 1024;
-    nst = MAX_STAGES;
-    while (nst > 2 && xbytes + (size_t)nst * G::STAGE_BYTES > budget) nst--;
-    smem = xbytes + (size_t)nst * G::STAGE_BYTES;
-  }
-  if (smem > budget) {
-    ctas_per_sm = 1;
-    while (nst < 4 && xbytes + (size_t)(nst + 1) * G::STAGE_BYTES <= full) nst++;
-    smem = xbytes + (size_t)nst * G::STAGE_BYTES;
-  }
-  return smem <= (size_t)d.max_smem;
+static bool plan8(const MmvqParams &p, int ncols, const DevInfo &d, int ctas_pref, LaunchPlan &lp) {
+  return plan_launch(Geo<T, 8, UPL>::S, QT<T>::QK, p.K, ncols, p.mode, p.vrows, 8, d.num_sms, d.max_smem, ctas_pref, lp);
 }
 
 template <int T, int NCOLS, bool FAST, int UPL>
 static cudaError_t launch_one(MmvqParams p, cudaStream_t stream) {
-  constexpr int NCW = 8, SLOTS = 2 * NCW;
+  constexpr int NCW = 8;
   const DevInfo &d = query_device();
-  int nst, ctas_per_sm;
-  size_t smem;
-  if (!plan8<T, UPL>(p, NCOLS, d, nst, smem, ctas_per_sm)) return cudaErrorInvalidConfiguration;
-  p.nstages = nst;
+  LaunchPlan lp;
+  if (!plan8<T, UPL>(p, NCOLS, d, g_ctas_per_sm, lp)) return cudaErrorInvalidConfiguration;
+  p.nstages = lp.nst;
   p.flags = g_flags;
 #ifdef MRS_TIMELINE
   p.dbg = (g_dbg != nullptr && g_dbg_launch < g_dbg_max) ? g_dbg + (size_t)(g_dbg_launch++) * 320 * 16 : nullptr;
 #endif
-  const int P = (p.mode == MODE_GLU) ? NCW : SLOTS;
-  int grid = (p.vrows + P - 1) / P;
-  const int max_grid = ctas_per_sm * d.num_sms;
-  if (grid > max_grid) grid = max_grid;
-  if (grid < 1) grid = 1;
   auto kern = mmvq_stream_kernel<T, NCOLS, FAST, NCW, UPL>;
   cudaFuncSetAttribute(kern, cudaFuncAttributeMaxDynamicSharedMemorySize, d.max_smem);
   cudaLaunchConfig_t cfg = {};
-  cfg.gridDim = dim3(grid);
+  cfg.gridDim = dim3(lp.grid);
   cfg.blockDim = dim3((NCW + 1) * 32);
-  cfg.dynamicSmemBytes = smem;
+  cfg.dynamicSmemBytes = lp.smem;
   cfg.stream = stream;
   cudaLaunchAttribute attr[1];
   attr[0].id = cudaLaunchAttributeProgrammaticStreamSerialization;
@@ -577,24 +551,23 @@
 template <int T1, int T2>
 static cudaError_t launch_dual(MmvqParams pa, MmvqParams pb, cudaStream_t stream) {
   const DevInfo &d = query_device();
-  int nsa, nsb, ca, cb;
-  size_t sma, smb;
+  LaunchPlan la, lb;
   if (pa.ncols != 1 || pb.ncols != 1 || !rows_aligned<T1>(pa) || !rows_aligned<T2>(pb) ||
-      !plan8<T1, QT<T1>::UPL>(pa, 1, d, nsa, sma, ca) || !plan8<T2, QT<T2>::UPL>(pb, 1, d, nsb, smb, cb) || ca < 2 || cb < 2)
+      !plan8<T1, QT<T1>::UPL>(pa, 1, d, g_ctas_per_sm, la) || !plan8<T2, QT<T2>::UPL>(pb, 1, d, g_ctas_per_sm, lb) ||
+      la.ctas_per_sm < 2 || lb.ctas_per_sm < 2)
     return cudaErrorNotSupported;
-  if (ca != 2 || cb != 2) {
-    const int keep = g_ctas_per_sm; g_ctas_per_sm = 2;
-    const bool ok = plan8<T1, QT<T1>::UPL>(pa, 1, d, nsa, sma, ca) && plan8<T2, QT<T2>::UPL>(pb, 1, d, nsb, smb, cb) && ca == 2 && cb == 2;
-    g_ctas_per_sm = keep;
-    if (!ok) return cudaErrorNotSupported;
-  }
-  pa.nstages = nsa; pb.nstages = nsb; pa.flags = pb.flags = g_flags;
+  if (la.ctas_per_sm != 2 || lb.ctas_per_sm != 2) {
+    if (!plan8<T1, QT<T1>::UPL>(pa, 1, d, 2, la) || !plan8<T2, QT<T2>::UPL>(pb, 1, d, 2, lb) || la.ctas_per_sm != 2 ||
+        lb.ctas_per_sm != 2)
+      return cudaErrorNotSupported;
+  }
+  pa.nstages = la.nst; pb.nstages = lb.nst; pa.flags = pb.flags = g_flags;
 #ifdef MRS_TIMELINE
   pa.dbg = (g_dbg != nullptr && g_dbg_launch < g_dbg_max) ? g_dbg + (size_t)(g_dbg_launch++) * 320 * 16 : nullptr;
   pb.dbg = pa.dbg;
 #endif
   const int slots = 2 * d.num_sms;
-  const int Pa = (pa.mode == MODE_GLU) ? 8 : 16, Pb = (pb.mode == MODE_GLU) ? 8 : 16;
+  const int Pa = plan_rows_per_pass(pa.mode, 8), Pb = plan_rows_per_pass(pb.mode, 8);
   int ga = (pa.vrows + Pa - 1) / Pa, gb = (pb.vrows + Pb - 1) / Pb;
   if (ga < 1 || gb < 1) return cudaErrorNotSupported;
   if (ga + gb > slots) {
@@ -606,7 +579,7 @@
   cudaLaunchConfig_t cfg = {};
   cfg.gridDim = dim3(ga + gb);
   cfg.blockDim = dim3(9 * 32);
-  cfg.dynamicSmemBytes = sma > smb ? sma : smb;
+  cfg.dynamicSmemBytes = la.smem > lb.smem ? la.smem : lb.smem;
   cfg.stream = stream;
   cudaLaunchAttribute attr[1];
   attr[0].id = cudaLaunchAttributeProgrammaticStreamSerialization;
@@ -625,20 +598,27 @@
 
 template <int T> struct HasLong { static constexpr bool value = (T == MRS_Q4_K || T == MRS_Q6_K); };
 
+template <int T> static bool takes_long(const MmvqParams &p, bool fast) {
+  if constexpr (HasLong<T>::value) {
+    const int row_bytes = (p.K / QT<T>::QK) * QT<T>::BYTES;
+    size_t wbytes = 0;
+    for (int m = 0; m < 3; m++)
+      if (p.w[m] != nullptr) wbytes += (size_t)p.nrows[m] * row_bytes;
+    return fast && p.ncols == 1 && !(g_flags & 8) && wbytes >= (size_t)g_long_min_bytes;
+  }
+  return false;
+}
+
 template <int T>
 static cudaError_t launch_type(MmvqParams p, cudaStream_t stream) {
   using Q = QT<T>;
   const bool fast = rows_aligned<T>(p);
-  const int row_bytes = (p.K / Q::QK) * Q::BYTES;
-  size_t wbytes = 0;
-  for (int m = 0; m < 3; m++)
-    if (p.w[m] != nullptr) wbytes += (size_t)p.nrows[m] * row_bytes;
+  const bool lng = takes_long<T>(p, fast);
   const int b = p.ncols;
 #define MRS_DISPATCH(NC)                                                                          \
   do {                                                                                            \
     if constexpr (HasLong<T>::value) {                                                            \
-      if (fast && NC == 1 && !(g_flags & 8) && wbytes >= (size_t)g_long_min_bytes)                \
-        return launch_one<T, NC, true, 2 * Q::UPL>(p, stream);                                    \
+      if (lng) return launch_one<T, NC, true, 2 * Q::UPL>(p, stream);                             \
     }                                                                                             \
     return fast ? launch_one<T, NC, true, Q::UPL>(p, stream) : launch_one<T, NC, false, Q::UPL>(p, stream); \
   } while (0)
@@ -647,6 +627,42 @@
   if (b <= 4) { MRS_DISPATCH(4); }
   MRS_DISPATCH(8);
 #undef MRS_DISPATCH
+}
+
+template <int T> static bool next_of(const MmvqParams &p, long long budget, MmvqNext &nx) {
+  const DevInfo &d = query_device();
+  const int nc = plan_ncols(p.ncols);
+  LaunchPlan lp;
+  bool ok;
+  if constexpr (HasLong<T>::value) {
+    ok = takes_long<T>(p, rows_aligned<T>(p)) ? plan8<T, 2 * QT<T>::UPL>(p, nc, d, g_ctas_per_sm, lp)
+                                              : plan8<T, QT<T>::UPL>(p, nc, d, g_ctas_per_sm, lp);
+  } else {
+    ok = plan8<T, QT<T>::UPL>(p, nc, d, g_ctas_per_sm, lp);
+  }
+  if (!ok) return false;
+  for (int m = 0; m < 3; m++) { nx.w[m] = p.w[m]; nx.nrows[m] = p.nrows[m]; }
+  nx.mode = p.mode; nx.vrows = p.vrows; nx.grid = lp.grid;
+  nx.row_bytes = (p.K / QT<T>::QK) * QT<T>::BYTES;
+  nx.lead = plan_lead(budget, nx.grid, nx.vrows, nx.mode, nx.row_bytes);
+  return true;
+}
+
+static bool mmvq_next_of(int type, const MmvqParams &p, long long budget, MmvqNext &nx) {
+  if (p.ncols < 1 || p.ncols > 8) return false;
+  switch (type) {
+  case MRS_Q4_0: return next_of<MRS_Q4_0>(p, budget, nx);
+  case MRS_Q4_1: return next_of<MRS_Q4_1>(p, budget, nx);
+  case MRS_Q5_0: return next_of<MRS_Q5_0>(p, budget, nx);
+  case MRS_Q5_1: return next_of<MRS_Q5_1>(p, budget, nx);
+  case MRS_Q8_0: return next_of<MRS_Q8_0>(p, budget, nx);
+  case MRS_Q2_K: return next_of<MRS_Q2_K>(p, budget, nx);
+  case MRS_Q3_K: return next_of<MRS_Q3_K>(p, budget, nx);
+  case MRS_Q4_K: return next_of<MRS_Q4_K>(p, budget, nx);
+  case MRS_Q5_K: return next_of<MRS_Q5_K>(p, budget, nx);
+  case MRS_Q6_K: return next_of<MRS_Q6_K>(p, budget, nx);
+  default: return false;
+  }
 }
 
 cudaError_t mmvq_dispatch(int type, const MmvqParams &p, cudaStream_t stream) {
@@ -777,19 +793,30 @@
 
 static cudaError_t mmvq_dispatch_dual_entry(int t1, const MmvqParams &pa, int t2, const MmvqParams &pb, cudaStream_t stream);
 
+static MmvqParams fused_params(const MmvqCall &c) {
+  MmvqParams p = {};
+  for (int m = 0; m < 3; m++) { p.w[m] = (const uint8_t *)c.w[m]; p.dst[m] = c.dst[m]; p.nrows[m] = c.n[m]; }
+  p.x = c.x; p.xkind = X_RAW; p.xdtype = c.dt; p.norm_w = c.norm_w; p.eps = c.eps; p.residual = c.residual;
+  p.K = c.K; p.stride_col_dst = c.n[0]; p.ncols = c.b_size; p.mode = c.mode; p.activation = c.activation;
+  p.dst_dtype = c.dt; p.pdl = c.pdl;
+  p.vrows = (c.mode == MODE_QKV) ? c.n[0] + c.n[1] + c.n[2] : c.n[0];
+  return p;
+}
+
 extern "C" int mrs_mmvq_fused(int ggml_type, int mode, int dt, const void *w0, const void *w1, const void *w2,
                               const void *x, const void *norm_w, float eps, const void *residual,
                               void *dst0, void *dst1, void *dst2, int K, int n0, int n1, int n2,
                               int b_size, int activation, int pdl, void *stream) {
-  MmvqParams p = {};
-  p.w[0] = (const uint8_t *)w0; p.w[1] = (const uint8_t *)w1; p.w[2] = (const uint8_t *)w2;
-  p.dst[0] = dst0; p.dst[1] = dst1; p.dst[2] = dst2;
-  p.nrows[0] = n0; p.nrows[1] = n1; p.nrows[2] = n2;
-  p.x = x; p.xkind = X_RAW; p.xdtype = dt; p.norm_w = norm_w; p.eps = eps; p.residual = residual;
-  p.K = K; p.stride_col_dst = n0; p.ncols = b_size; p.mode = mode; p.activation = activation;
-  p.dst_dtype = dt; p.pdl = pdl;
-  p.vrows = (mode == MODE_QKV) ? n0 + n1 + n2 : n0;
-  return (int)mmvq_dispatch(ggml_type, p, (cudaStream_t)stream);
+  const MmvqCall c = {ggml_type, mode, dt, {w0, w1, w2}, x, norm_w, eps, residual, {dst0, dst1, dst2}, K, {n0, n1, n2},
+                      b_size, activation, pdl};
+  return (int)mmvq_dispatch(ggml_type, fused_params(c), (cudaStream_t)stream);
+}
+
+cudaError_t mrs::mmvq_fused_call(const MmvqCall &c, const MmvqCall *next, bool idle, cudaStream_t stream) {
+  MmvqParams p = fused_params(c);
+  const long long budget = idle ? L2_PREFETCH_IDLE_BYTES : L2_PREFETCH_BYTES;
+  if (next != nullptr && !mmvq_next_of(next->type, fused_params(*next), budget, p.next)) p.next = MmvqNext{};
+  return mmvq_dispatch(c.type, p, stream);
 }
 
 static cudaError_t mmvq_dispatch_dual_entry(int t1, const MmvqParams &pa, int t2, const MmvqParams &pb, cudaStream_t stream) {
diff --git a/mistral.rs_b200/csrc/mmvq_call.cuh b/mistral.rs_b200/csrc/mmvq_call.cuh
--- /dev/null
+++ b/mistral.rs_b200/csrc/mmvq_call.cuh
@@ -0,0 +1,18 @@
+#pragma once
+#include <cuda_runtime.h>
+
+namespace mrs {
+
+struct MmvqCall {
+  int type, mode, dt;
+  const void *w[3];
+  const void *x, *norm_w;
+  float eps;
+  const void *residual;
+  void *dst[3];
+  int K, n[3], b_size, activation, pdl;
+};
+
+cudaError_t mmvq_fused_call(const MmvqCall &c, const MmvqCall *next, bool idle, cudaStream_t stream);
+
+}
diff --git a/mistral.rs_b200/csrc/mmvq_plan.cuh b/mistral.rs_b200/csrc/mmvq_plan.cuh
--- /dev/null
+++ b/mistral.rs_b200/csrc/mmvq_plan.cuh
@@ -0,0 +1,128 @@
+#pragma once
+#include <stddef.h>
+#include <stdint.h>
+
+#if defined(__CUDACC__)
+#define MRS_PLAN_FN __host__ __device__ __forceinline__
+#else
+#define MRS_PLAN_FN inline
+#endif
+
+namespace mrs {
+
+enum { MODE_PLAIN = 0, MODE_GLU = 1, MODE_QKV = 2 };
+
+constexpr int MAX_STAGES = 12;
+
+#ifndef MRS_L2_PREFETCH_BYTES
+#define MRS_L2_PREFETCH_BYTES (8ll << 20)
+#endif
+#ifndef MRS_L2_PREFETCH_IDLE_BYTES
+#define MRS_L2_PREFETCH_IDLE_BYTES (40ll << 20)
+#endif
+constexpr long long L2_PREFETCH_BYTES = MRS_L2_PREFETCH_BYTES;
+constexpr long long L2_PREFETCH_IDLE_BYTES = MRS_L2_PREFETCH_IDLE_BYTES;
+
+struct SegGeo {
+  int seg_units, seg_blocks, seg_bytes, slot_bytes, stage_bytes, xu_bytes;
+};
+MRS_PLAN_FN constexpr SegGeo seg_geo(int blk_bytes, int upb, int aux, int upl, int ncw) {
+  return SegGeo{32 * upl, 32 * upl / upb, (32 * upl / upb) * blk_bytes,
+                ((32 * upl / upb) * blk_bytes + 30 + 15) & ~15,
+                2 * ncw * (((32 * upl / upb) * blk_bytes + 30 + 15) & ~15), 32 + 4 * aux};
+}
+
+MRS_PLAN_FN int plan_rows_per_pass(int mode, int ncw) { return mode == MODE_GLU ? ncw : 2 * ncw; }
+MRS_PLAN_FN int plan_vrow_mats(int mode) { return mode == MODE_GLU ? 2 : 1; }
+MRS_PLAN_FN int plan_ncols(int b) { return b == 1 ? 1 : b == 2 ? 2 : b <= 4 ? 4 : 8; }
+
+struct LaunchPlan {
+  int nst;
+  int ctas_per_sm;
+  int grid;
+  size_t smem;
+};
+
+MRS_PLAN_FN bool plan_launch(const SegGeo &g, int qk, int K, int ncols, int mode, int vrows, int ncw, int num_sms,
+                             int max_smem, int ctas_pref, LaunchPlan &lp) {
+  const int nblocks = K / qk;
+  const int nseg = (nblocks + g.seg_blocks - 1) / g.seg_blocks;
+  const int npos = nseg * g.seg_units;
+  const size_t xbytes = 256 + (size_t)ncols * npos * g.xu_bytes + 128;
+  const size_t stage = (size_t)g.stage_bytes;
+  int ctas = (ncols == 1) ? ctas_pref : (ctas_pref > 2 ? 2 : ctas_pref);
+  size_t budget = (size_t)max_smem / (ctas < 2 ? 2 : ctas) - 1024;
+  const size_t full = (size_t)max_smem - 1024;
+  int nst = MAX_STAGES;
+  while (nst > 2 && xbytes + (size_t)nst * stage > budget) nst--;
+  size_t smem = xbytes + (size_t)nst * stage;
+  if (smem > budget && ctas == 3) {
+    ctas = 2;
+    budget = (size_t)max_smem / 2 - 1024;
+    nst = MAX_STAGES;
+    while (nst > 2 && xbytes + (size_t)nst * stage > budget) nst--;
+    smem = xbytes + (size_t)nst * stage;
+  }
+  if (smem > budget) {
+    ctas = 1;
+    while (nst < 4 && xbytes + (size_t)(nst + 1) * stage <= full) nst++;
+    smem = xbytes + (size_t)nst * stage;
+  }
+  const int P = plan_rows_per_pass(mode, ncw);
+  int grid = (vrows + P - 1) / P;
+  if (grid > ctas * num_sms) grid = ctas * num_sms;
+  if (grid < 1) grid = 1;
+  lp.nst = nst; lp.ctas_per_sm = ctas; lp.grid = grid; lp.smem = smem;
+  return smem <= (size_t)max_smem;
+}
+
+MRS_PLAN_FN void plan_cta_rows(int vrows, int cta, int ncta, int &vr0, int &vr1) {
+  vr0 = (int)((long long)vrows * cta / ncta);
+  vr1 = (int)((long long)vrows * (cta + 1) / ncta);
+}
+
+MRS_PLAN_FN void plan_resolve_row(int mode, const int *nrows, int vrow, int which, int &m, int &row) {
+  if (mode == MODE_QKV) {
+    if (vrow < nrows[0]) { m = 0; row = vrow; }
+    else if (vrow < nrows[0] + nrows[1]) { m = 1; row = vrow - nrows[0]; }
+    else { m = 2; row = vrow - nrows[0] - nrows[1]; }
+  } else if (mode == MODE_GLU) {
+    m = which; row = vrow;
+  } else {
+    m = 0; row = vrow;
+  }
+}
+
+MRS_PLAN_FN void plan_granules(uintptr_t a, uint32_t len, uintptr_t &a0, uint32_t &bytes) {
+  a0 = a & ~(uintptr_t)15;
+  bytes = (uint32_t)(((a + len + 15) & ~(uintptr_t)15) - a0);
+}
+
+struct MmvqNext {
+  const uint8_t *w[3];
+  int nrows[3];
+  int mode, vrows, row_bytes, grid;
+  int lead;
+};
+
+MRS_PLAN_FN int plan_lead(long long budget, int grid, int vrows, int mode, int row_bytes) {
+  const long long per = (long long)grid * plan_vrow_mats(mode) * (row_bytes + 32);
+  const long long lead = per > 0 ? budget / per : 0;
+  const int most = grid > 0 ? (vrows + grid - 1) / grid : 0;
+  return lead < most ? (int)lead : most;
+}
+
+MRS_PLAN_FN int plan_prefetch_items(const MmvqNext &nx, int j, int &vr0) {
+  int vr1;
+  plan_cta_rows(nx.vrows, j, nx.grid, vr0, vr1);
+  const int n = vr1 - vr0 < nx.lead ? vr1 - vr0 : nx.lead;
+  return n * plan_vrow_mats(nx.mode);
+}
+MRS_PLAN_FN void plan_prefetch_item(const MmvqNext &nx, int vr0, int i, uintptr_t &a0, uint32_t &bytes) {
+  const int nm = plan_vrow_mats(nx.mode);
+  int m, row;
+  plan_resolve_row(nx.mode, nx.nrows, vr0 + i / nm, i % nm, m, row);
+  plan_granules((uintptr_t)(nx.w[m] + (size_t)row * nx.row_bytes), (uint32_t)nx.row_bytes, a0, bytes);
+}
+
+}
```

Measured after the change: 370.7, median of 6. 1.03x the previous value.
